# Orion-AI-Lab/KuroSiwo

Hardware: AMD Instinct MI355X
Metric: SAR tiles/sec (224x224, SNUNet-ECAM change-detection train step) (higher is better)
Workload: dtype bf16; 1 GPU; BASELINE.json configs[1]: SNUNet-ECAM CD, 2 dates x 2-ch GRD 224x224, per-GPU batch 32, ce+dice loss, Adam lr 1e-3, fwd+loss+bwd+optimizer; global_batch=32, base_channel=32, parallelism=dp1, hip_streams=3

## Files before the change

### include/ksmi.h

```cpp
#ifndef KSMI_H
#define KSMI_H
#include <stddef.h>
#include <stdint.h>

#ifdef __cplusplus
extern "C" {
#endif

#define KSMI_ABI_VERSION 7
#define KSMI_F32 0
#define KSMI_BF16 1
#define KSMI_E_ARG (-1)
#define KSMI_E_UNSUPPORTED (-2)
#define KSMI_MAX_SRC 6
#define KSMI_MAX_CHUNKS 72

int ksmi_abi_version(void);
const char* ksmi_last_error(void);
int ksmi_set_knob(const char* name, const char* value);
int ksmi_chunk_elems(int dtype);

#define KSMI_OP_CALL 0
#define KSMI_OP_ORDER 1
#define KSMI_OP_WAIT_SIDE 2
// ... 26 lines not shown
  int32_t n_begin;
  int32_t n_len;
  int32_t accumulate;
  int32_t pad_;
} ksmi_dst;

typedef struct ksmi_conv_desc {
  ksmi_src src[KSMI_MAX_SRC];
  ksmi_dst dst[KSMI_MAX_SRC];
  int32_t nsrc, ndst;
  const void* wpk;
  const float* bias;
  float* stats;
  const void* mask_src;
  const float* m_mean; const float* m_rstd; const float* m_scale; const float* m_shift;
  int32_t B, Hin, Win, Hout, Wout;
  int32_t KH, KW, stride, pad;
  int32_t TH, TW;
  int32_t N, Npad;
  int32_t nchunks;
  int32_t ps_cout;
  uint16_t chunk_c0[KSMI_MAX_CHUNKS];
  uint8_t chunk_src[KSMI_MAX_CHUNKS];
  int32_t pad_x;
  int32_t out_sy, out_sx, out_oy, out_ox, out_H, out_W;
  int32_t uniform_kc;
  int32_t in_sy, in_sx, in_oy, in_ox, in_H, in_W;
  float alpha;
  int32_t relu_out;
  int32_t residC;
  const void* resid;
  int32_t stats_rows;
  const void* gate_src; const void* xhat_src; const float* g_mean; const float* g_rstd;
  int32_t dir;
  int32_t pad2_;
} ksmi_conv_desc;


int ksmi_last_kernels(char* buf, int cap);
int ksmi_hbm_probe(int mode, const void* a, void* b, void* c, size_t nbytes, unsigned* sink, void* stream);
size_t ksmi_desc_size(int which);
int ksmi_conv_gate_supported(const ksmi_conv_desc* d, int dtype);
int ksmi_conv_grid_m(const ksmi_conv_desc* d);
int ksmi_conv_stats_rows(const ksmi_conv_desc* d, int dtype);
int ksmi_conv_forward(const ksmi_conv_desc* d, int dtype, void* stream);
int ksmi_conv_dispatch_info(const ksmi_conv_desc* d, int dtype, int32_t* info);

typedef struct ksmi_pack_desc {
  const float* w; void* out;
  int32_t nchunks, taps, N, Npad, n_mod;
  int64_t sK, sN, sD, sT;
  int32_t flip;
  int32_t k_off[KSMI_MAX_CHUNKS];
  int32_t k_len[KSMI_MAX_CHUNKS];
  int32_t use_tap_map;
  int32_t tap_map[16];
  int32_t uniform_kc, k_total;
} ksmi_pack_desc;
int ksmi_pack_weights(const ksmi_pack_desc* d, int dtype, void* stream);
int ksmi_pack_weights_batched(const ksmi_pack_desc* descs_device, int n, int dtype, void* stream);

typedef struct ksmi_wgrad_desc {
  ksmi_src src[KSMI_MAX_SRC];
  int32_t nsrc;
  const void* dy; int32_t dyC; int32_t dy_c_off;
  int32_t B, Hin, Win, Hout, Wout;
  int32_t KH, KW, stride, pad;
  int32_t TH, TW;
  int32_t N;
  int32_t nchunks;
  int32_t nsplit;
  float* partial;
  float* grad; int64_t gK, gN, gT; int32_t accumulate;
  int32_t k_off[KSMI_MAX_CHUNKS];
  int32_t k_len[KSMI_MAX_CHUNKS];
  uint16_t chunk_c0[KSMI_MAX_CHUNKS];
  uint8_t chunk_src[KSMI_MAX_CHUNKS];
  int32_t uniform_kc, k_total;
  int32_t in_sy, in_sx, in_oy, in_ox, in_H, in_W;
  int32_t pad_x_set, pad_x;
  int32_t use_tap_off;
  int32_t tap_off[16];
  float* bias_grad; int32_t bias_accumulate;
} ksmi_wgrad_desc;
size_t ksmi_conv_wgrad_workspace(const ksmi_wgrad_desc* d, int dtype);
int ksmi_conv_wgrad(const ksmi_wgrad_desc* d, int dtype, void* stream);
int ksmi_conv_wgrad_fuses_bias(const ksmi_wgrad_desc* d, int dtype);

int ksmi_conv_first_forward(const float* x_nchw, const float* w, const float* bias, void* out, float* stats,
                            int B, int Cin, int H, int W, int Cout, int dtype, void* stream);
int ksmi_conv_first_forward_raw(const float* x_nchw, const float* x_tail, int c_head, const float* w, const float* bias,
                                void* out, float* stats, int B, int Cin, int H, int W, int Cout, const float* mean,
                                const float* stdv, const float* clamp, int dtype, void* stream);
int ksmi_conv_first_stats_rows(int B, int H, int W);
int ksmi_im2col3x3(const float* x_nchw, void* out, int B, int Cin, int H, int W, int Kpad, int dtype, void* stream);
int ksmi_im2col3x3_raw(const float* x_nchw, const float* x_tail, int c_head, void* out, int B, int Cin, int H, int W,
                       int Kpad, const float* mean, const float* stdv, const float* clamp, int dtype, void* stream);
int ksmi_conv_first_wgrad(const float* x_nchw, const void* dy, float* dw, float* workspace, size_t ws_bytes,
                          int B, int Cin, int H, int W, int Cout, int accumulate, int dtype, void* stream);
size_t ksmi_conv_first_wgrad_workspace(int B, int Cin, int H, int W, int Cout);

int ksmi_bn_finalize(const float* partial, int rows, int Cpad, int C, double count,
                     const float* gamma, const float* beta, float* running_mean, float* running_var,
                     int64_t* num_batches_tracked, float momentum, float eps, int training,
                     float* mean, float* rstd, float* scale, float* shift, void* stream);
int ksmi_bn_add_relu(const void* z, const void* identity, const float* scale, const float* shift, void* out,
                     int64_t npix, int C, int dtype, void* stream);
int ksmi_bnrelu_bwd_reduce(const void* dout, const void* out, const void* z, const float* mean, const float* rstd,
                           float* partial, int rows, int64_t npix, int C, int dtype, void* stream);
int ksmi_reduce_rows(const float* partial, int rows, int K, int Cstride, int C, float* sums,
                     float* dgamma, float* dbeta, int accumulate, void* stream);
typedef struct ksmi_rowsum_desc {
  const float* partial;
  float* dst;
  int32_t rows, K, k, Cstride, C, accumulate;
  int32_t head, next;
} ksmi_rowsum_desc;
int ksmi_reduce_rows_batched(const ksmi_rowsum_desc* descs_device, int n, void* stream);
int ksmi_reduce_rows_batched_wide(const ksmi_rowsum_desc* descs_device, int n, int max_c, void* stream);
int ksmi_bnrelu_bwd_apply(void* dout_g, const void* out, const void* z, const float* mean, const float* rstd,
                          const float* gamma, const float* sums, void* dz, double count,
                          int64_t npix, int C, int dtype, void* stream);
int ksmi_bn_bwd_apply_gated(const void* g, const void* z, const float* mean, const float* rstd, const float* gamma, const float* sums,
                            void* dz, double count, int64_t npix, int C, int dtype, void* stream);
int ksmi_bn_bwd_apply_add(void* r_di, const void* g, const void* i, const float* mean, const float* rstd,
                          const float* gamma, const float* sums, float* partial, int rows, double count,
                          int64_t npix, int C, int dtype, void* stream);
int ksmi_bn_fused_supported(int C, int Cstride, int dtype);
int ksmi_bn_fused_max_rows(void);
int ksmi_bn_fin_add_relu(float* partial, int rows, int Cpad, int C, double count, const float* gamma, const float* beta,
                         float* running_mean, float* running_var, int64_t* num_batches_tracked, float momentum, float eps,
                         float* mean, float* rstd, float* scale, float* shift, const void* z, const void* identity, void* out,
                         void* pooled, int B, int H, int W, int dtype, void* stream);
int ksmi_bn_bwd_fin_apply_gated(float* partial, int rows, int Cstride, float* sums, float* dgamma, float* dbeta, int accumulate,
                                const void* g, const void* z, const float* mean, const float* rstd, const float* gamma, void* dz,
                                double count, int64_t npix, int C, int dtype, void* stream);
int ksmi_bnrelu_bwd_fin_apply(float* partial, int rows, int Cstride, float* sums, float* dgamma, float* dbeta, int accumulate,
                              void* dout_g, const void* out, const void* z, const float* mean, const float* rstd, const float* gamma,
                              void* dz, double count, int64_t npix, int C, int dtype, void* stream);
int ksmi_bn_bwd_fin_apply_add(float* partial, int rows, int Cstride, float* sums, float* dgamma, float* dbeta, int accumulate,
                              void* r_di, const void* g, const void* i, const float* mean, const float* rstd, const float* gamma,
                              float* bias_partial, int bias_rows, double count, int64_t npix, int C, int dtype, void* stream);
int ksmi_channel_sum(const void* x, float* partial, int rows, int64_t npix, int C, int dtype, void* stream);
int ksmi_colsum(const void* x, int64_t rows, int C, float* out, int accumulate, int dtype, void* stream);

int ksmi_maxpool2x2_forward(const void* x, void* y, int B, int H, int W, int C, int dtype, void* stream);
int ksmi_maxpool2x2_backward(const void* x, const void* dy, void* dx, int accumulate,
                             int B, int H, int W, int C, int dtype, void* stream);

int ksmi_ecam_pool(const void* const x[4], float* avg, float* mx, int32_t* argmax,
                   float* workspace, int B, int HW, int C, int dtype, void* stream);
size_t ksmi_ecam_pool_workspace(int B, int HW, int C);
int ksmi_ecam_mlp(const float* avg, const float* mx, const float* ca_fc1, const float* ca_fc2,
                  const float* ca1_fc1, const float* ca1_fc2, float* ca, float* ca1,
                  float* hidden , int B, int C, void* stream);
int ksmi_ecam_final_forward(const void* const x[4], const float* ca, const float* ca1, const float* wf,
                            const float* bias, float* logits, int B, int HW, int C, int ncls, int dtype, void* stream);
int ksmi_ecam_final_backward_reduce(const void* const x[4], const float* dlogits, const float* ca, const float* ca1,
                                    const float* wf, float* dca, float* dca1, float* dwf, float* dbias,
                                    float* workspace, int B, int HW, int C, int ncls, int dtype, void* stream);
size_t ksmi_ecam_bwd_workspace(int B, int HW, int C, int ncls);
int ksmi_ecam_mlp_backward(const float* avg, const float* mx, const float* hidden, const float* ca, const float* ca1,
                           const float* dca, const float* dca1, const float* ca_fc1, const float* ca_fc2,
                           const float* ca1_fc1, const float* ca1_fc2, float* davg, float* dmax,
                           float* g_ca_fc1, float* g_ca_fc2, float* g_ca1_fc1, float* g_ca1_fc2,
                           float* workspace, int B, int C, void* stream);
size_t ksmi_ecam_mlp_bwd_workspace(int B, int C);
int ksmi_ecam_final_backward_dx(void* const dx[4], const float* dlogits, const float* ca, const float* wf,
                                const float* davg, const float* dmax, const int32_t* argmax,
                                int B, int HW, int C, int ncls, int dtype, void* stream);

size_t ksmi_loss_workspace(int B, int HW);
int ksmi_ce_dice_forward(const float* logits, const int64_t* labels, const float* class_w, int with_dice,
                         float* out3, float* workspace, int B, int HW, int ignore_index, void* stream);
int ksmi_ce_dice_backward(const float* logits, const int64_t* labels, const float* class_w, int with_dice,
                          const float* workspace, const float* grad_scale ,
                          float* dlogits, int B, int HW, int ignore_index, void* stream);

#define KSMI_LOSS_DICE 1
#define KSMI_LOSS_LOVASZ 2
// ... 181 lines not shown
```

### kurosiwo_amd/_lib.py

```python
import ctypes as C
import os

_HERE = os.path.dirname(os.path.abspath(__file__))
LIB_PATH = os.path.join(_HERE, "libksmi.so")

KSMI_F32, KSMI_BF16 = 0, 1
LOSS_DICE, LOSS_LOVASZ, LOSS_FOCAL = 1, 2, 3
MAX_SRC, MAX_CHUNKS = 6, 72
ABI_VERSION = 7


class KsmiError(RuntimeError):
    pass


class Src(C.Structure):
    _fields_ = [("ptr", C.c_void_p), ("scale", C.c_void_p), ("shift", C.c_void_p),
                ("C", C.c_int32), ("c_off", C.c_int32), ("c_len", C.c_int32), ("relu", C.c_int32)]


class Dst(C.Structure):
    _fields_ = [("ptr", C.c_void_p), ("C", C.c_int32), ("c_off", C.c_int32), ("n_begin", C.c_int32),
                ("n_len", C.c_int32), ("accumulate", C.c_int32), ("pad_", C.c_int32)]


class ConvDesc(C.Structure):
    _fields_ = [("src", Src * MAX_SRC), ("dst", Dst * MAX_SRC), ("nsrc", C.c_int32), ("ndst", C.c_int32),
                ("wpk", C.c_void_p), ("bias", C.c_void_p), ("stats", C.c_void_p),
                ("mask_src", C.c_void_p), ("m_mean", C.c_void_p), ("m_rstd", C.c_void_p),
                ("m_scale", C.c_void_p), ("m_shift", C.c_void_p),
                ("B", C.c_int32), ("Hin", C.c_int32), ("Win", C.c_int32), ("Hout", C.c_int32), ("Wout", C.c_int32),
                ("KH", C.c_int32), ("KW", C.c_int32), ("stride", C.c_int32), ("pad", C.c_int32),
                ("TH", C.c_int32), ("TW", C.c_int32), ("N", C.c_int32), ("Npad", C.c_int32),
                ("nchunks", C.c_int32), ("ps_cout", C.c_int32),
                ("chunk_c0", C.c_uint16 * MAX_CHUNKS), ("chunk_src", C.c_uint8 * MAX_CHUNKS),
                ("pad_x", C.c_int32), ("out_sy", C.c_int32), ("out_sx", C.c_int32), ("out_oy", C.c_int32),
                ("out_ox", C.c_int32), ("out_H", C.c_int32), ("out_W", C.c_int32),
                ("uniform_kc", C.c_int32), ("in_sy", C.c_int32), ("in_sx", C.c_int32), ("in_oy", C.c_int32), ("in_ox", C.c_int32),
                ("in_H", C.c_int32), ("in_W", C.c_int32), ("alpha", C.c_float), ("relu_out", C.c_int32), ("residC", C.c_int32),
                ("resid", C.c_void_p), ("stats_rows", C.c_int32),
                ("gate_src", C.c_void_p), ("xhat_src", C.c_void_p), ("g_mean", C.c_void_p), ("g_rstd", C.c_void_p),
                ("dir", C.c_int32), ("pad2_", C.c_int32)]


class PackDesc(C.Structure):
    _fields_ = [("w", C.c_void_p), ("out", C.c_void_p),
                ("nchunks", C.c_int32), ("taps", C.c_int32), ("N", C.c_int32), ("Npad", C.c_int32), ("n_mod", C.c_int32),
                ("sK", C.c_int64), ("sN", C.c_int64), ("sD", C.c_int64), ("sT", C.c_int64),
                ("flip", C.c_int32),
                ("k_off", C.c_int32 * MAX_CHUNKS), ("k_len", C.c_int32 * MAX_CHUNKS),
                ("use_tap_map", C.c_int32), ("tap_map", C.c_int32 * 16), ("uniform_kc", C.c_int32), ("k_total", C.c_int32)]


class TiffInfo(C.Structure):
    _fields_ = [(k, C.c_int32) for k in ("width", "height", "bands", "bits", "sample_format", "compression", "predictor", "tiled",
                                         "big_endian", "bigtiff", "has_geo", "has_nodata")] + [
        ("pixel_scale", C.c_double * 2), ("origin", C.c_double * 2), ("tie_pixel", C.c_double * 2), ("nodata", C.c_double)]


class RowsumDesc(C.Structure):
    _fields_ = [("partial", C.c_void_p), ("dst", C.c_void_p), ("rows", C.c_int32), ("K", C.c_int32), ("k", C.c_int32),
                ("Cstride", C.c_int32), ("C", C.c_int32), ("accumulate", C.c_int32), ("head", C.c_int32), ("next", C.c_int32)]


class WgradDesc(C.Structure):
    _fields_ = [("src", Src * MAX_SRC), ("nsrc", C.c_int32),
                ("dy", C.c_void_p), ("dyC", C.c_int32), ("dy_c_off", C.c_int32),
                ("B", C.c_int32), ("Hin", C.c_int32), ("Win", C.c_int32), ("Hout", C.c_int32), ("Wout", C.c_int32),
                ("KH", C.c_int32), ("KW", C.c_int32), ("stride", C.c_int32), ("pad", C.c_int32),
                ("TH", C.c_int32), ("TW", C.c_int32), ("N", C.c_int32), ("nchunks", C.c_int32), ("nsplit", C.c_int32),
                ("partial", C.c_void_p), ("grad", C.c_void_p),
                ("gK", C.c_int64), ("gN", C.c_int64), ("gT", C.c_int64), ("accumulate", C.c_int32),
                ("k_off", C.c_int32 * MAX_CHUNKS), ("k_len", C.c_int32 * MAX_CHUNKS),
                ("chunk_c0", C.c_uint16 * MAX_CHUNKS), ("chunk_src", C.c_uint8 * MAX_CHUNKS),
                ("uniform_kc", C.c_int32), ("k_total", C.c_int32),
                ("in_sy", C.c_int32), ("in_sx", C.c_int32), ("in_oy", C.c_int32), ("in_ox", C.c_int32), ("in_H", C.c_int32), ("in_W", C.c_int32),
                ("pad_x_set", C.c_int32), ("pad_x", C.c_int32), ("use_tap_off", C.c_int32), ("tap_off", C.c_int32 * 16),
                ("bias_grad", C.c_void_p), ("bias_accumulate", C.c_int32)]


class Op(C.Structure):
    _fields_ = [(k, C.c_int32) for k in ("kind", "sig", "lane", "side", "tag", "a", "b", "nargs")] + [("fn", C.c_void_p), ("args", C.c_void_p)]


OP_CALL, OP_ORDER, OP_WAIT_SIDE = 0, 1, 2

_vp, _i, _i64, _f, _d, _sz = C.c_void_p, C.c_int, C.c_int64, C.c_float, C.c_double, C.c_size_t
_P4 = C.c_void_p * 4

SIGNATURES = {
    "ksmi_abi_version": (_i, []),
    "ksmi_last_kernels": (_i, [C.c_char_p, _i]),
    "ksmi_hbm_probe": (_i, [_i, _vp, _vp, _vp, C.c_size_t, _vp, _vp]),
    "ksmi_last_error": (C.c_char_p, []),
    "ksmi_set_knob": (_i, [C.c_char_p, C.c_char_p]),
    "ksmi_thunk_id": (_i, [C.c_char_p]),
    "ksmi_runner_create": (_vp, []),
    "ksmi_runner_destroy": (_i, [_vp]),
    "ksmi_runner_set_streams": (_i, [_vp, _vp, _vp, _vp, _vp]),
    "ksmi_run_list": (_i, [_vp, _vp, _i, _i, _vp, C.POINTER(C.c_int32)]),
    "ksmi_runner_join": (_i, [_vp]),
    "ksmi_conv_dispatch_info": (_i, [C.POINTER(ConvDesc), _i, C.POINTER(C.c_int32)]),
    "ksmi_chunk_elems": (_i, [_i]),
    "ksmi_conv_grid_m": (_i, [C.POINTER(ConvDesc)]),
    "ksmi_conv_forward": (_i, [C.POINTER(ConvDesc), _i, _vp]),
    "ksmi_pack_weights": (_i, [C.POINTER(PackDesc), _i, _vp]),
    "ksmi_pack_weights_batched": (_i, [_vp, _i, _i, _vp]),
    "ksmi_conv_wgrad_workspace": (_sz, [C.POINTER(WgradDesc), _i]),
    "ksmi_conv_wgrad": (_i, [C.POINTER(WgradDesc), _i, _vp]),
    "ksmi_conv_wgrad_fuses_bias": (_i, [C.POINTER(WgradDesc), _i]),
    "ksmi_conv_stats_rows": (_i, [C.POINTER(ConvDesc), _i]),
    "ksmi_conv_gate_supported": (_i, [C.POINTER(ConvDesc), _i]),
    "ksmi_desc_size": (C.c_size_t, [_i]),
    "ksmi_conv_first_forward": (_i, [_vp, _vp, _vp, _vp, _vp, _i, _i, _i, _i, _i, _i, _vp]),
    "ksmi_conv_first_forward_raw": (_i, [_vp, _vp, _i, _vp, _vp, _vp, _vp, _i, _i, _i, _i, _i, _vp, _vp, _vp, _i, _vp]),
    "ksmi_conv_first_stats_rows": (_i, [_i, _i, _i]),
    "ksmi_im2col3x3": (_i, [_vp, _vp, _i, _i, _i, _i, _i, _i, _vp]),
    "ksmi_im2col3x3_raw": (_i, [_vp, _vp, _i, _vp, _i, _i, _i, _i, _i, _vp, _vp, _vp, _i, _vp]),
    "ksmi_conv_first_wgrad": (_i, [_vp, _vp, _vp, _vp, _sz, _i, _i, _i, _i, _i, _i, _i, _vp]),
    "ksmi_conv_first_wgrad_workspace": (_sz, [_i, _i, _i, _i, _i]),
    "ksmi_bn_finalize": (_i, [_vp, _i, _i, _i, _d, _vp, _vp, _vp, _vp, _vp, _f, _f, _i, _vp, _vp, _vp, _vp, _vp]),
    "ksmi_bn_add_relu": (_i, [_vp, _vp, _vp, _vp, _vp, _i64, _i, _i, _vp]),
    "ksmi_bn_fused_supported": (_i, [_i, _i, _i]),
    "ksmi_bn_fused_max_rows": (_i, []),
    "ksmi_bn_fin_add_relu": (_i, [_vp, _i, _i, _i, _d, _vp, _vp, _vp, _vp, _vp, _f, _f, _vp, _vp, _vp, _vp, _vp, _vp, _vp, _vp, _i, _i, _i, _i, _vp]),
    "ksmi_bn_bwd_fin_apply_gated": (_i, [_vp, _i, _i, _vp, _vp, _vp, _i, _vp, _vp, _vp, _vp, _vp, _vp, _d, _i64, _i, _i, _vp]),
    "ksmi_bnrelu_bwd_fin_apply": (_i, [_vp, _i, _i, _vp, _vp, _vp, _i, _vp, _vp, _vp, _vp, _vp, _vp, _vp, _d, _i64, _i, _i, _vp]),
    "ksmi_bn_bwd_fin_apply_add": (_i, [_vp, _i, _i, _vp, _vp, _vp, _i, _vp, _vp, _vp, _vp, _vp, _vp, _vp, _i, _d, _i64, _i, _i, _vp]),
    "ksmi_bnrelu_bwd_reduce": (_i, [_vp, _vp, _vp, _vp, _vp, _vp, _i, _i64, _i, _i, _vp]),
    "ksmi_reduce_rows": (_i, [_vp, _i, _i, _i, _i, _vp, _vp, _vp, _i, _vp]),
    "ksmi_reduce_rows_batched": (_i, [_vp, _i, _vp]),
    "ksmi_reduce_rows_batched_wide": (_i, [_vp, _i, _i, _vp]),
    "ksmi_bnrelu_bwd_apply": (_i, [_vp, _vp, _vp, _vp, _vp, _vp, _vp, _vp, _d, _i64, _i, _i, _vp]),
    "ksmi_bn_bwd_apply_gated": (_i, [_vp, _vp, _vp, _vp, _vp, _vp, _vp, _d, _i64, _i, _i, _vp]),
    "ksmi_bn_bwd_apply_add": (_i, [_vp, _vp, _vp, _vp, _vp, _vp, _vp, _vp, _i, _d, _i64, _i, _i, _vp]),
    "ksmi_channel_sum": (_i, [_vp, _vp, _i, _i64, _i, _i, _vp]),
    "ksmi_colsum": (_i, [_vp, _i64, _i, _vp, _i, _i, _vp]),
    "ksmi_gather_rows": (_i, [_vp, _vp, _i, _vp, _vp, _i, _i, _i, _i, _i, _i, _vp]),
    "ksmi_scatter_rows": (_i, [_vp, _vp, _vp, _i, _vp, _vp, _i, _i, _i, _i, _i, _vp]),
    "ksmi_batch_sum": (_i, [_vp, _vp, _i, _i64, _i, _i, _vp]),
    "ksmi_mse_workspace": (C.c_size_t, []),
    "ksmi_mse_loss": (_i, [_vp, _vp, _vp, _f, _vp, _vp, _vp, _i64, _i, _vp]),
    "ksmi_maxpool2x2_forward": (_i, [_vp, _vp, _i, _i, _i, _i, _i, _vp]),
    "ksmi_maxpool2x2_backward": (_i, [_vp, _vp, _vp, _i, _i, _i, _i, _i, _i, _vp]),
    "ksmi_ecam_pool": (_i, [_P4, _vp, _vp, _vp, _vp, _i, _i, _i, _i, _vp]),
    "ksmi_ecam_pool_workspace": (_sz, [_i, _i, _i]),
    "ksmi_ecam_mlp": (_i, [_vp, _vp, _vp, _vp, _vp, _vp, _vp, _vp, _vp, _i, _i, _vp]),
    "ksmi_ecam_final_forward": (_i, [_P4, _vp, _vp, _vp, _vp, _vp, _i, _i, _i, _i, _i, _vp]),
    "ksmi_ecam_final_backward_reduce": (_i, [_P4, _vp, _vp, _vp, _vp, _vp, _vp, _vp, _vp, _vp, _i, _i, _i, _i, _i, _vp]),
    "ksmi_ecam_bwd_workspace": (_sz, [_i, _i, _i, _i]),
    "ksmi_ecam_mlp_backward": (_i, [_vp] * 18 + [_i, _i, _vp]),
    "ksmi_ecam_mlp_bwd_workspace": (_sz, [_i, _i]),
    "ksmi_ecam_final_backward_dx": (_i, [_P4, _vp, _vp, _vp, _vp, _vp, _vp, _i, _i, _i, _i, _i, _vp]),
    "ksmi_loss_workspace": (_sz, [_i, _i]),
    "ksmi_ce_dice_forward": (_i, [_vp, _vp, _vp, _i, _vp, _vp, _i, _i, _i, _vp]),
    "ksmi_ce_dice_backward": (_i, [_vp, _vp, _vp, _i, _vp, _vp, _vp, _i, _i, _i, _vp]),
    "ksmi_seg_loss_workspace": (_sz, [_i, _i, _i]),
    "ksmi_seg_loss_forward": (_i, [_i, _vp, _vp, _vp, _f, _vp, _vp, _i, _i, _i, _vp]),
    "ksmi_seg_loss_backward": (_i, [_i, _vp, _vp, _vp, _f, _vp, _vp, _vp, _i, _i, _i, _vp]),
    "ksmi_argmax_confusion": (_i, [_vp, _vp, _vp, _vp, _i, _i, _i, _i, _vp]),
    "ksmi_argmax_confusion_grouped": (_i, [_vp, _vp, _vp, _vp, _vp, _vp, _vp, _vp, _i, _i, _i, _i, _vp]),
    "ksmi_adam_step": (_i, [_vp, _vp, _vp, _vp, _i64, _vp, _f, _f, _f, _f, _f, _f, _vp]),
    "ksmi_adamw_step": (_i, [_vp, _vp, _vp, _vp, _i64, _vp, _f, _f, _f, _f, _f, _f, _vp]),
    "ksmi_adam_step_mirror": (_i, [_vp, _vp, _vp, _vp, _i64, _vp, _f, _f, _f, _f, _f, _f, _i, _vp, _vp]),
    "ksmi_sgd_step": (_i, [_vp, _vp, _vp, _i64, _vp, _f, _f, _f, _f, _vp]),
    "ksmi_layernorm_forward": (_i, [_vp, _vp, _vp, _vp, _vp, _vp, _i, _i, _f, _i, _vp]),
    "ksmi_layernorm_bwd_blocks": (_i, [_i]),
    "ksmi_layernorm_backward": (_i, [_vp, _vp, _vp, _vp, _vp, _vp, _i, _vp, _i, _i, _i, _vp]),
    "ksmi_gelu_forward": (_i, [_vp, _vp, _i64, _i, _vp]),
    "ksmi_gelu_backward": (_i, [_vp, _vp, _vp, _i64, _i, _vp]),
    "ksmi_add": (_i, [_vp, _vp, _vp, _i64, _i, _vp]),
    "ksmi_relu_backward": (_i, [_vp, _vp, _vp, _i64, _i, _vp]),
    "ksmi_relu_forward": (_i, [_vp, _vp, _i64, _i, _vp]),
    "ksmi_sar_preprocess": (_i, [_vp, _vp, _vp, _vp, _i, _i, _i64, C.c_float, _vp]),
    "ksmi_augment_views": (_i, [_vp, _vp, _vp, _vp, _vp, _vp, _i, _i, _i, _i, _f, C.c_uint32, _f, _f, C.c_uint32, _f, _f, C.c_uint32, _i, _i, _i, _i, _vp, _vp]),
    "ksmi_augment_masks": (_i, [_vp, _vp, _vp, _vp, _vp, _i, _i, _i, _i, _vp]),
    "ksmi_bmm_f32": (_i, [_vp, _vp, _vp, _vp, _i, _i, _i, _i, _i, C.POINTER(C.c_int64), C.POINTER(C.c_int64), C.POINTER(C.c_int64), C.c_float, _i, _vp]),
    "ksmi_softmax_rows_f32": (_i, [_vp, _vp, _i64, _i, C.c_float, _vp]),
    "ksmi_softmax_rows_backward_f32": (_i, [_vp, _vp, _vp, _i64, _i, C.c_float, _vp]),
    "ksmi_semantic_tokens_forward": (_i, [_vp, _vp, _vp, _vp, _vp, _i, _i, _i, _i, _i, _i, _vp]),
    "ksmi_semantic_tokens_backward": (_i, [_vp, _vp, _vp, _vp, _vp, _vp, _i, _i, _i, _i, _i, _i, _i, _vp]),
    "ksmi_token_cross_forward": (_i, [_vp, _vp, _vp, _vp, _vp, _vp, _vp, _i, _i, _i, _i, _i, _i, C.c_float, _i, _vp]),
    "ksmi_token_cross_bwd_workspace": (_sz, [_i, _i, _i]),
    "ksmi_token_cross_backward": (_i, [_vp, _vp, _vp, _vp, _vp, _vp, _vp, _vp, _vp, _vp, _vp, _i, _i, _vp, _i, _i, _i, _i, _i, _i, C.c_float, _i, _vp]),
    "ksmi_tiff_info_read": (_i, [C.c_char_p, C.POINTER(TiffInfo)]),
    "ksmi_tiff_read_f32": (_i, [C.c_char_p, _vp, _i64, C.POINTER(TiffInfo)]),
    "ksmi_tiff_read_native": (_i, [C.c_char_p, _vp, _i64, C.POINTER(TiffInfo)]),
    "ksmi_tile_batch_read": (_i, [C.POINTER(C.c_char_p), _i, _vp, _i, _i, _i]),
    "ksmi_tile_batch_read_bands": (_i, [C.POINTER(C.c_char_p), _i, _vp, _i, _i, _i, _i]),
    "ksmi_tiles_fill_nodata": (_i, [_vp, _i, _i, _i, _i]),
    "ksmi_cast_bf16": (_i, [_vp, _vp, _i64, _vp]),
    "ksmi_up_gemm_supported": (_i, [_i, _i, _i, _i, _i]),
    "ksmi_up_wgrad_supported": (_i, [_i, _i, _i, _i, _i]),
    "ksmi_up_pack_weight": (_i, [_vp, _vp, _i, _vp]),
    "ksmi_up_pack_weights_batched": (_i, [_vp, _vp, _vp, _i, _vp]),
    "ksmi_up_forward": (_i, [_vp, _vp, _vp, _vp, _i, _i, _i, _i, _vp]),
    "ksmi_up_dgrad": (_i, [_vp, _vp, _vp, _i, _i, _i, _i, _i, _vp]),
    "ksmi_up_wgrad_workspace": (C.c_size_t, [_i, _i, _i, _i]),
    "ksmi_up_wgrad": (_i, [_vp, _vp, _vp, _vp, _i, _i, _i, _i, _i, _vp]),
    "ksmi_gemm_nt": (_i, [_vp, _i, _vp, _i, _vp, _vp, _i, _vp, _i, _i, _i, _i, _vp]),
    "ksmi_gemm_nn": (_i, [_vp, _i, _vp, _i, _vp, _i, _i, _i, _i, _i, _vp]),
# ... 114 lines not shown
```

### kurosiwo_amd/csrc/elementwise.hip

```cpp
#include <stdlib.h>
#include "common.h"
#include "../../include/ksmi.h"
#include "errors.h"

namespace {

constexpr int kThreads = 256;

struct ChanWalk {
  int cv, pl, npl, active;
  __device__ ChanWalk(int CV) {
    npl = kThreads / CV; if (npl < 1) npl = 1;
    active = (int)threadIdx.x < npl * CV && CV <= kThreads;
    cv = threadIdx.x % CV; pl = threadIdx.x / CV;
  }
};

template <int K, int VEC>
__device__ __forceinline__ void block_channel_reduce(const float* val, const ChanWalk& w, int CV, int C, float* partial, int row) {
  __shared__ float red[kThreads * 2];
#pragma unroll
  for (int k = 0; k < K; ++k) {
#pragma unroll
    for (int j0 = 0; j0 < VEC; j0 += 2) {
// ... 450 lines not shown
  for (int c = 0; c < CIN; ++c)
#pragma unroll
    for (int t = 0; t < 9; ++t) xin[c * 9 + t] = xs[c * 324 + (ly + t / 3) * 18 + lx + t % 3];
  for (int n0 = 0; n0 < Cout; n0 += NC) {
    const int nc = min(NC, Cout - n0);
    for (int i = tid; i < nc * KTP; i += 256) { const int j = i / KTP, k = i - j * KTP; wl[i] = k < KT ? w[(n0 + j) * KT + k] : 0.f; }
    if (tid < nc) wl[NC * KTP + tid] = bias ? bias[n0 + tid] : 0.f;
    __syncthreads();
#pragma unroll 4
    for (int j = 0; j < nc; ++j) {
      float a = wl[NC * KTP + j];
      float wr[KTP];
#pragma unroll
      for (int k = 0; k < KTP; k += 4) *(f32x4*)(wr + k) = *(const f32x4*)(wl + j * KTP + k);
#pragma unroll
      for (int k = 0; k < KT; ++k) a = fmaf(xin[k], wr[k], a);
      ot[tid * OP + j] = ok ? ElemTraits<T>::cvt(a) : 0.f;
    }
    __syncthreads();
    if (stats) {
      const int n = tid & (NC - 1), grp = tid / NC;
      if (n < nc) {
        float sm = 0.f, sq = 0.f;
#pragma unroll 8
        for (int i = 0; i < NC; ++i) { const float v = ot[(grp * NC + i) * OP + n]; sm += v; sq += v * v; }
        red[(grp * 2 + 0) * NC + n] = sm; red[(grp * 2 + 1) * NC + n] = sq;
      }
    }
    const int vpp = nc / VEC;
    for (int v = tid; v < 256 * vpp; v += 256) {
      const int p = v / vpp, q = v - p * vpp;
      const int py = ty * 16 + (p >> 4), px = tx * 16 + (p & 15);
      if (py >= H || px >= W) continue;
      float o[VEC];
#pragma unroll
      for (int j = 0; j < VEC; ++j) o[j] = ot[p * OP + q * VEC + j];
      *(u32x4*)(out + (((int64_t)b * H + py) * W + px) * Cout + n0 + q * VEC) = vec_pack<T>(o);
    }
    __syncthreads();
    if (stats && tid < 2 * nc) {
      const int which = tid / nc, n = tid - which * nc;
      float t = 0.f;
#pragma unroll
      for (int g = 0; g < G; ++g) t += red[(g * 2 + which) * NC + n];
      stats[((size_t)blockIdx.x * 2 + which) * Cout + n0 + n] = t;
    }
  }
}

template <typename T>
__global__ __launch_bounds__(256) void im2col3x3_kernel(const float* __restrict__ x, T* out, int B, int Cin, int H, int W, int Kpad,
                                                        const float* __restrict__ nmean, const float* __restrict__ nstd,
                                                        const float* __restrict__ nclamp, const float* __restrict__ xtail, int chead) {
  constexpr int VEC = ElemTraits<T>::kVec;
  extern __shared__ __attribute__((aligned(16))) unsigned char smem[];
  float* xs = (float*)smem;
  const int tilesX = (W + 15) / 16, tilesY = (H + 15) / 16;
  int bm = blockIdx.x;
  const int tx = bm % tilesX; bm /= tilesX;
  const int ty = bm % tilesY; const int b = bm / tilesY;
  const int tid = threadIdx.x;
  for (int i = tid; i < Cin * 324; i += 256) {
    const int c = i / 324, r = i - c * 324, hy = r / 18, hx = r - hy * 18;
    const int iy = ty * 16 - 1 + hy, ix = tx * 16 - 1 + hx;
    float v = 0.f;
    if (iy >= 0 && iy < H && ix >= 0 && ix < W) v = raw_tile_value(image_value(x, xtail, chead, Cin, b, c, H, W, iy, ix), c, nmean, nstd, nclamp);
    xs[i] = v;
  }
  __syncthreads();
  const int KV = Kpad / VEC;
  for (int v = tid; v < 256 * KV; v += 256) {
    const int p = v / KV, q = v - p * KV;
    const int ly = p >> 4, lx = p & 15;
    const int oy = ty * 16 + ly, ox = tx * 16 + lx;
    if (oy >= H || ox >= W) continue;
    float f[VEC];
#pragma unroll
    for (int j = 0; j < VEC; ++j) {
      const int k = q * VEC + j;
      const int c = k / 9, t = k - c * 9;
      f[j] = c < Cin ? xs[c * 324 + (ly + t / 3) * 18 + lx + t % 3] : 0.f;
    }
    *(u32x4*)(out + (((int64_t)b * H + oy) * W + ox) * Kpad + q * VEC) = vec_pack<T>(f);
  }
}

template <typename T>
__global__ __launch_bounds__(256) void conv_first_wgrad_kernel(const float* x, const T* dy, float* partial,
                                                               int B, int Cin, int H, int W, int Cout) {
  extern __shared__ __attribute__((aligned(16))) unsigned char smem[];
  float* xs = (float*)smem;
  float* dys = xs + Cin * 324;
  const int tilesX = (W + 15) / 16, tilesY = (H + 15) / 16;
  const int patches = B * tilesX * tilesY;
  const int tid = threadIdx.x;
  const int KT = Cin * 9;
  const int n = tid % Cout, grp = tid / Cout, ngrp = 256 / Cout;
  constexpr int MAXK = 12;
  float acc[MAXK];
#pragma unroll
  for (int j = 0; j < MAXK; ++j) acc[j] = 0.f;
  const int ldy = Cout + 1;
  for (int patch = blockIdx.x; patch < patches; patch += gridDim.x) {
    int bm = patch;
    const int tx = bm % tilesX; bm /= tilesX;
    const int ty = bm % tilesY; const int b = bm / tilesY;
    __syncthreads();
    for (int i = tid; i < Cin * 324; i += 256) {
      const int c = i / 324, r = i - c * 324, hy = r / 18, hx = r - hy * 18;
      const int iy = ty * 16 - 1 + hy, ix = tx * 16 - 1 + hx;
      xs[i] = (iy >= 0 && iy < H && ix >= 0 && ix < W) ? x[(((int64_t)b * Cin + c) * H + iy) * W + ix] : 0.f;
    }
    for (int i = tid; i < 256 * Cout; i += 256) {
      const int p = i / Cout, nn = i - p * Cout;
      const int oy = ty * 16 + (p >> 4), ox = tx * 16 + (p & 15);
      dys[p * ldy + nn] = (oy < H && ox < W) ? ElemTraits<T>::ld(dy + (((int64_t)b * H + oy) * W + ox) * Cout + nn) : 0.f;
    }
    __syncthreads();
    for (int p = 0; p < 256; ++p) {
      const float g = dys[p * ldy + n];
      const int ly = p >> 4, lx = p & 15;
#pragma unroll
      for (int j = 0; j < MAXK; ++j) {
        const int k = grp + j * ngrp;
        if (k < KT) {
          const int c = k / 9, t = k - c * 9;
          acc[j] += g * xs[c * 324 + (ly + t / 3) * 18 + lx + t % 3];
        }
      }
    }
  }
#pragma unroll
  for (int j = 0; j < MAXK; ++j) {
    const int k = grp + j * ngrp;
    if (k < KT) partial[((size_t)blockIdx.x * Cout + n) * KT + k] = acc[j];
  }
}

__global__ void sum_rows_flat_kernel(const float* partial, int rows, int64_t n, float* out, int accumulate) {
  for (int64_t i = (int64_t)blockIdx.x * blockDim.x + threadIdx.x; i < n; i += (int64_t)gridDim.x * blockDim.x) {
    double s = 0.0;
    for (int r = 0; r < rows; ++r) s += (double)partial[(size_t)r * n + i];
    out[i] = accumulate ? out[i] + (float)s : (float)s;
  }
}

__global__ void step_increment_kernel(int64_t* step) { if (threadIdx.x == 0 && blockIdx.x == 0) *step += 1; }

template <bool DECOUPLED, bool MIRROR = false>
__global__ void adam_kernel(float* p, const float* g, float* m, float* v, int64_t n, const int64_t* step,
                            float lr, float b1, float b2, float eps, float wd, float gscale, bf16_t* mirror = nullptr) {
  const double t = (double)*step;
  const float bc1 = (float)(1.0 - pow((double)b1, t));
  const float bc2s = (float)sqrt(1.0 - pow((double)b2, t));
  const float step_size = lr / bc1;
  auto upd = [&](float gi, float& pi, float& mi, float& vi) {
    gi *= gscale;
    if (DECOUPLED) pi = pi * (1.f - lr * wd);
    else if (wd != 0.f) gi += wd * pi;
    mi = mi + (gi - mi) * (1.f - b1);
    vi = vi * b2 + gi * gi * (1.f - b2);
    const float denom = sqrtf(vi) / bc2s + eps;
    pi = pi - step_size * (mi / denom);
  };
  const bool vec = ((((uintptr_t)p | (uintptr_t)g | (uintptr_t)m | (uintptr_t)v) & 15) == 0);
  const int64_t nv = vec ? n / 4 : 0;
// ... 318 lines not shown

int ksmi_conv_first_stats_rows(int B, int H, int W) { return B * ((H + 15) / 16) * ((W + 15) / 16); }

static int first_conv_sources(const float* xtail, int* chead, int Cin, const float* nmean, const float* nstd, const float* nclamp) {
  if ((nmean != nullptr) != (nstd != nullptr) || (nmean != nullptr) != (nclamp != nullptr))
    return ksmi_fail(KSMI_E_ARG, "conv_first: mean, std and clamp come together");
  if (xtail == nullptr) *chead = Cin;
  else if (*chead < 1 || *chead >= Cin) return ksmi_fail(KSMI_E_ARG, "conv_first: a tail image needs 1 <= c_head < Cin");
  return 0;
}

int ksmi_conv_first_forward_raw(const float* x, const float* xtail, int chead, const float* w, const float* bias, void* out, float* stats,
                                int B, int Cin, int H, int W, int Cout, const float* nmean, const float* nstd, const float* nclamp,
                                int dtype, void* stream) {
  if (int rc = first_conv_sources(xtail, &chead, Cin, nmean, nstd, nclamp)) return rc;
  const int vec = dtype == KSMI_BF16 ? 8 : 4;
  if (Cin < 1 || Cin > 8 || Cout % vec || Cout > 256) return ksmi_fail(KSMI_E_ARG, "conv_first: Cin<=8, Cout multiple of vector, <=256");
  const int grid = ksmi_conv_first_stats_rows(B, H, W);
  const size_t lds = (size_t)(Cin * 324 + 256 * 17 + 512 + 16 * ((Cin * 9 + 3) / 4 * 4) + 16) * sizeof(float);
  hipStream_t st = (hipStream_t)stream;
#define KSMI_CF(CIN_)                                                                                                     \
  case CIN_:                                                                                                              \
    if (dtype == KSMI_BF16) hipLaunchKernelGGL((conv_first_fwd_kernel<bf16_t, CIN_>), dim3(grid), dim3(256), lds, st, x, w, bias, (bf16_t*)out, stats, B, H, W, Cout, nmean, nstd, nclamp, xtail, chead); \
    else hipLaunchKernelGGL((conv_first_fwd_kernel<float, CIN_>), dim3(grid), dim3(256), lds, st, x, w, bias, (float*)out, stats, B, H, W, Cout, nmean, nstd, nclamp, xtail, chead);                    \
    break;
  if (dtype != KSMI_BF16 && dtype != KSMI_F32) return ksmi_fail(KSMI_E_ARG, "bad dtype");
  switch (Cin) { KSMI_CF(1) KSMI_CF(2) KSMI_CF(3) KSMI_CF(4) KSMI_CF(5) KSMI_CF(6) KSMI_CF(7) KSMI_CF(8) }
#undef KSMI_CF
  return ksmi_check_launch("conv_first_fwd");
}

int ksmi_conv_first_forward(const float* x, const float* w, const float* bias, void* out, float* stats, int B, int Cin, int H,
                            int W, int Cout, int dtype, void* stream) {
  return ksmi_conv_first_forward_raw(x, nullptr, Cin, w, bias, out, stats, B, Cin, H, W, Cout, nullptr, nullptr, nullptr, dtype, stream);
}

static int conv_first_wgrad_blocks(int B, int H, int W) {
  const int patches = B * ((H + 15) / 16) * ((W + 15) / 16);
  return patches < 512 ? patches : 512;
}

size_t ksmi_conv_first_wgrad_workspace(int B, int Cin, int H, int W, int Cout) {
  return (size_t)conv_first_wgrad_blocks(B, H, W) * Cout * Cin * 9 * sizeof(float);
}

int ksmi_conv_first_wgrad(const float* x, const void* dy, float* dw, float* workspace, size_t ws_bytes, int B, int Cin, int H,
                          int W, int Cout, int accumulate, int dtype, void* stream) {
  if (Cin < 1 || Cin > 8 || 256 % Cout || (Cin * 9 + 256 / Cout - 1) / (256 / Cout) > 12)
    return ksmi_fail(KSMI_E_ARG, "conv_first_wgrad: unsupported Cin/Cout");
  if (ws_bytes < ksmi_conv_first_wgrad_workspace(B, Cin, H, W, Cout)) return ksmi_fail(KSMI_E_ARG, "conv_first_wgrad: workspace too small");
  const int blocks = conv_first_wgrad_blocks(B, H, W);
  const size_t lds = (size_t)(Cin * 324 + 256 * (Cout + 1)) * sizeof(float);
  KSMI_DT(dtype,
          {
            auto k = conv_first_wgrad_kernel<bf16_t>;
            if (lds > 65536) (void)hipFuncSetAttribute((const void*)k, hipFuncAttributeMaxDynamicSharedMemorySize, (int)lds);
            hipLaunchKernelGGL(k, dim3(blocks), dim3(256), lds, (hipStream_t)stream, x, (const bf16_t*)dy, workspace, B, Cin, H, W, Cout);
          },
          {
            auto k = conv_first_wgrad_kernel<float>;
            if (lds > 65536) (void)hipFuncSetAttribute((const void*)k, hipFuncAttributeMaxDynamicSharedMemorySize, (int)lds);
            hipLaunchKernelGGL(k, dim3(blocks), dim3(256), lds, (hipStream_t)stream, x, (const float*)dy, workspace, B, Cin, H, W, Cout);
          });
  int rc = ksmi_check_launch("conv_first_wgrad");
  if (rc) return rc;
  const int64_t n = (int64_t)Cout * Cin * 9;
  hipLaunchKernelGGL(sum_rows_flat_kernel, dim3(grid_for(n)), dim3(256), 0, (hipStream_t)stream, workspace, blocks, n, dw, accumulate);
  return ksmi_check_launch("conv_first_wgrad_reduce");
}

int ksmi_im2col3x3_raw(const float* x_nchw, const float* xtail, int chead, void* out, int B, int Cin, int H, int W, int Kpad,
                       const float* nmean, const float* nstd, const float* nclamp, int dtype, void* stream) {
  if (int rc = first_conv_sources(xtail, &chead, Cin, nmean, nstd, nclamp)) return rc;
  const int vec = dtype == KSMI_BF16 ? 8 : 4;
  if (Cin < 1 || Cin * 9 > Kpad || Kpad % vec || Cin > 32) return ksmi_fail(KSMI_E_ARG, "im2col3x3: need Cin*9 <= Kpad, Kpad multiple of the vector");
  const int grid = B * ((H + 15) / 16) * ((W + 15) / 16);
  const size_t lds = (size_t)Cin * 324 * sizeof(float);
  KSMI_DT(dtype,
          hipLaunchKernelGGL(im2col3x3_kernel<bf16_t>, dim3(grid), dim3(256), lds, (hipStream_t)stream, x_nchw, (bf16_t*)out, B, Cin, H, W, Kpad, nmean, nstd, nclamp, xtail, chead),
          hipLaunchKernelGGL(im2col3x3_kernel<float>, dim3(grid), dim3(256), lds, (hipStream_t)stream, x_nchw, (float*)out, B, Cin, H, W, Kpad, nmean, nstd, nclamp, xtail, chead));
  return ksmi_check_launch("im2col3x3");
}

int ksmi_im2col3x3(const float* x_nchw, void* out, int B, int Cin, int H, int W, int Kpad, int dtype, void* stream) {
  return ksmi_im2col3x3_raw(x_nchw, nullptr, Cin, out, B, Cin, H, W, Kpad, nullptr, nullptr, nullptr, dtype, stream);
}

int ksmi_adam_step(float* p, const float* g, float* m, float* v, int64_t n, int64_t* step_count, float lr, float beta1,
                   float beta2, float eps, float weight_decay, float grad_scale, void* stream) {
  if (!p || !g || !m || !v || !step_count || n < 0) return ksmi_fail(KSMI_E_ARG, "adam: bad args");
  hipLaunchKernelGGL(step_increment_kernel, dim3(1), dim3(64), 0, (hipStream_t)stream, step_count);
  hipLaunchKernelGGL((adam_kernel<false, false>), dim3(grid_for((n + 3) / 4, 8192)), dim3(256), 0, (hipStream_t)stream, p, g, m, v, n, step_count, lr, beta1,
                     beta2, eps, weight_decay, grad_scale, (bf16_t*)nullptr);
  return ksmi_check_launch("adam");
}

int ksmi_adam_step_mirror(float* p, const float* g, float* m, float* v, int64_t n, int64_t* step_count, float lr, float beta1,
                          float beta2, float eps, float weight_decay, float grad_scale, int decoupled, void* mirror_bf16, void* stream) {
  if (!p || !g || !m || !v || !step_count || !mirror_bf16 || n < 0 || ((uintptr_t)mirror_bf16 & 7)) return ksmi_fail(KSMI_E_ARG, "adam_mirror: bad args");
  hipLaunchKernelGGL(step_increment_kernel, dim3(1), dim3(64), 0, (hipStream_t)stream, step_count);
  if (decoupled)
    hipLaunchKernelGGL((adam_kernel<true, true>), dim3(grid_for((n + 3) / 4, 8192)), dim3(256), 0, (hipStream_t)stream, p, g, m, v, n, step_count, lr, beta1,
                       beta2, eps, weight_decay, grad_scale, (bf16_t*)mirror_bf16);
  else
    hipLaunchKernelGGL((adam_kernel<false, true>), dim3(grid_for((n + 3) / 4, 8192)), dim3(256), 0, (hipStream_t)stream, p, g, m, v, n, step_count, lr, beta1,
                       beta2, eps, weight_decay, grad_scale, (bf16_t*)mirror_bf16);
  return ksmi_check_launch("adam_mirror");
}

int ksmi_adamw_step(float* p, const float* g, float* m, float* v, int64_t n, int64_t* step_count, float lr, float beta1,
                    float beta2, float eps, float weight_decay, float grad_scale, void* stream) {
  if (!p || !g || !m || !v || !step_count || n < 0) return ksmi_fail(KSMI_E_ARG, "adamw: bad args");
  hipLaunchKernelGGL(step_increment_kernel, dim3(1), dim3(64), 0, (hipStream_t)stream, step_count);
  hipLaunchKernelGGL((adam_kernel<true, false>), dim3(grid_for((n + 3) / 4, 8192)), dim3(256), 0, (hipStream_t)stream, p, g, m, v, n, step_count, lr, beta1,
                     beta2, eps, weight_decay, grad_scale, (bf16_t*)nullptr);
  return ksmi_check_launch("adamw");
}

int ksmi_sgd_step(float* p, const float* g, float* mom, int64_t n, int64_t* step_count, float lr, float momentum,
                  float weight_decay, float grad_scale, void* stream) {
  if (!p || !g || !step_count || (momentum != 0.f && !mom)) return ksmi_fail(KSMI_E_ARG, "sgd: bad args");
  hipLaunchKernelGGL(step_increment_kernel, dim3(1), dim3(64), 0, (hipStream_t)stream, step_count);
  hipLaunchKernelGGL(sgd_kernel, dim3(grid_for(n, 4096)), dim3(256), 0, (hipStream_t)stream, p, g, mom, n, step_count, lr, momentum,
                     weight_decay, grad_scale);
  return ksmi_check_launch("sgd");
}

int ksmi_fill_zero(void* p, size_t bytes, void* stream) {
  hipError_t e = hipMemsetAsync(p, 0, bytes, (hipStream_t)stream);
  if (e != hipSuccess) return ksmi_fail((int)e, hipGetErrorString(e));
  return 0;
}

int ksmi_nchw_to_nhwc(const float* x, void* y, int B, int C, int HW, int dtype, void* stream) {
  const int64_t n = (int64_t)B * C * HW;
  KSMI_DT(dtype,
          hipLaunchKernelGGL(nchw_to_nhwc_kernel<bf16_t>, dim3(grid_for(n, 8192)), dim3(256), 0, (hipStream_t)stream, x, (bf16_t*)y, B, C, HW),
          hipLaunchKernelGGL(nchw_to_nhwc_kernel<float>, dim3(grid_for(n, 8192)), dim3(256), 0, (hipStream_t)stream, x, (float*)y, B, C, HW));
  return ksmi_check_launch("nchw_to_nhwc");
}

int ksmi_nhwc_to_nchw(const void* x, float* y, int B, int C, int HW, int dtype, void* stream) {
  const int64_t n = (int64_t)B * C * HW;
  KSMI_DT(dtype,
          hipLaunchKernelGGL(nhwc_to_nchw_kernel<bf16_t>, dim3(grid_for(n, 8192)), dim3(256), 0, (hipStream_t)stream, (const bf16_t*)x, y, B, C, HW),
          hipLaunchKernelGGL(nhwc_to_nchw_kernel<float>, dim3(grid_for(n, 8192)), dim3(256), 0, (hipStream_t)stream, (const float*)x, y, B, C, HW));
  return ksmi_check_launch("nhwc_to_nchw");
}

int ksmi_selftest_mma(const void* a, const void* b, float* c, int dtype, void* stream) {
  KSMI_DT(dtype,
          hipLaunchKernelGGL(selftest_mma_kernel<bf16_t>, dim3(1), dim3(64), 0, (hipStream_t)stream, (const bf16_t*)a, (const bf16_t*)b, c),
          hipLaunchKernelGGL(selftest_mma_kernel<float>, dim3(1), dim3(64), 0, (hipStream_t)stream, (const float*)a, (const float*)b, c));
  return ksmi_check_launch("selftest_mma");
}

int ksmi_selftest_tr16(const uint16_t* in256, uint16_t* out256, void* stream) {
  hipLaunchKernelGGL(selftest_tr16_kernel, dim3(1), dim3(64), 0, (hipStream_t)stream, in256, out256);
  return ksmi_check_launch("selftest_tr16");
}

}
```

### kurosiwo_amd/csrc/igemm.hip

```cpp
#include <stdio.h>
#include <stdlib.h>
#include "common.h"
#include "../../include/ksmi.h"
#include "errors.h"
#include "igemm_epilogue.h"
#include "wgrad3.h"
#include "igemm3.h"
#include "igemm4.h"

namespace {


template <typename T, int NT, int KH, int KW>
__global__ __launch_bounds__(256) void igemm_fwd_kernel(const ksmi_conv_desc d) {
  constexpr int TAPS = KH * KW;
  constexpr int BN = NT * 16;
  constexpr int VEC = ElemTraits<T>::kVec;
  constexpr int KC = VEC * 4;
  extern __shared__ __attribute__((aligned(16))) unsigned char smem[];

  const int tid = threadIdx.x, lane = tid & 63, wave = tid >> 6;
  const int g = lane >> 4, l15 = lane & 15;

  const int tilesX = (d.Wout + d.TW - 1) / d.TW, tilesY = (d.Hout + d.TH - 1) / d.TH;
// ... 690 lines not shown
static bool wgrad_generic_forced() { static const bool on = ksmi_knob_is_set("KSMI_WGRAD_GENERIC"); return on; }
static bool gemm_tn_eligible(const ksmi_wgrad_desc* d, int es) {
  return es == 2 && d->KH == 1 && d->KW == 1 && d->stride == 1 && d->pad == 0 && d->nsrc == 1 && d->src[0].scale == nullptr &&
         d->Hin == d->Hout && d->Win == d->Wout && (d->src[0].c_len % 8) == 0 && (d->N % 8) == 0 && d->N >= 64 && d->src[0].c_len >= 64 &&
         !wgrad_generic_forced();
}
static void gemm_tn_geom(const ksmi_wgrad_desc* d, int kc, int& nsplit, int& rps, int& tk, int& tn, int& bt) {
  const int rows = d->B * d->Hout * d->Wout;
  const int K = d->nchunks * kc;
  const int npad = (d->N + 15) & ~15;
  tk = (K + 127) / 128; tn = (npad + 127) / 128;
  bool plain = d->gK == 1 && (!d->use_tap_off || d->tap_off[0] == 0) && d->gN >= d->src[0].c_len && d->gN < ((int64_t)1 << 31);
  if (plain && !d->uniform_kc)
    for (int i = 0; i < d->nchunks; ++i) plain = plain && d->k_off[i] == i * kc;
  const int steps_all = (rows + 63) / 64;
  double best = 1e30; int bs = 1; bt = 128;
  static const int f_bt = ksmi_knob_int("KSMI_TN_BT", 0), f_s = ksmi_knob_int("KSMI_TN_SPLIT", 0);
  for (int b = 128; b >= 64; b -= 32) {
    if (f_bt && b != f_bt) continue;
    const double step_us = b == 128 ? 0.95 : b == 96 ? 0.78 : 0.6;
    for (int s = 1; s <= 256 && s <= steps_all; s = s < 8 ? s + 1 : s * 2) {
      if (s == 1 && !plain) continue;
      if (f_s && s != f_s) continue;
      const int acols = s == 1 ? K : npad, bcols = s == 1 ? npad : K;
      const int tiles = ((acols + 127) / 128) * ((bcols + b - 1) / b);
      const int steps = (steps_all + s - 1) / s;
      const int rounds = (tiles * s + 255) / 256;
      const bool spl = ksmi_gemm2_tn_spl(tiles * s, steps);
      double t = rounds * ((spl ? 0.73 : 1.0) * steps * step_us + (spl ? 4.0 : 3.0));
      if (s > 1) t += 2.0 * s * (double)K * npad * 4.0 / 4.0e6 + 3.0 + 0.08 * (s > 16 ? 16 + (s - 16) / 8 : s);
      if (t < best) { best = t; bs = s; bt = b; }
    }
  }
  rps = ((steps_all + bs - 1) / bs) * 64;
  nsplit = (rows + rps - 1) / rps;
}

struct WgradGeom { int taps, kc, nt, bn, patches, pps, nsplit, ntiles, npad; size_t lds; bool tn; int rps, tk, tnn, tbt; bool v3; ksmi_wgrad3_geom_t g3; };

template <typename T>
WgradGeom wgrad_geom(const ksmi_wgrad_desc* d) {
  WgradGeom g;
  g.taps = d->KH * d->KW;
  g.kc = ElemTraits<T>::kVec * 4;
  g.npad = (d->N + 15) & ~15;
  g.nt = g.npad >= 64 ? 4 : (g.npad >= 32 ? 2 : 1);
  static const int wnt_cap = ksmi_knob_int("KSMI_WGRAD_NT", 4);
  if (g.nt > wnt_cap) g.nt = wnt_cap;
  static const bool wnt4 = ksmi_knob_is_set("KSMI_WGRAD_NT4");
  if (g.taps >= 9 && g.nt > 2 && !wnt4) g.nt = 2;
  g.bn = g.nt * 16;
  g.ntiles = (g.npad + g.bn - 1) / g.bn;
  const int tilesX = (d->Wout + d->TW - 1) / d->TW, tilesY = (d->Hout + d->TH - 1) / d->TH;
  g.patches = d->B * tilesX * tilesY;
  static const int wg_target = ksmi_knob_int("KSMI_WGRAD_WGS", 1024);
  static const int split_cap = ksmi_knob_int("KSMI_WGRAD_SPLITS", 512);
  int want = wg_target / (d->nchunks * g.ntiles);
  if (want < 1) want = 1;
  if (want > split_cap) want = split_cap;
  if (want > g.patches) want = g.patches;
  g.pps = (g.patches + want - 1) / want;
  g.nsplit = (g.patches + g.pps - 1) / g.pps;
  const int HH = (d->TH - 1) * d->stride + d->KH, HW = (d->TW - 1) * d->stride + d->KW;
  const int P = d->TH * d->TW, Ppad = (P + g.kc - 1) / g.kc * g.kc;
  g.lds = ((HH * HW * 64 + 255) & ~255) + (size_t)Ppad * g.bn * sizeof(T);
  if (g.taps == 1 && g.lds < (size_t)(g.kc / 16) * g.nt * 4096) g.lds = (size_t)(g.kc / 16) * g.nt * 4096;
  g.tn = gemm_tn_eligible(d, (int)sizeof(T));
  if (g.tn) gemm_tn_geom(d, g.kc, g.nsplit, g.rps, g.tk, g.tnn, g.tbt);
  g.v3 = !g.tn && ksmi_wgrad3_geom(d, sizeof(T) == 2 ? KSMI_BF16 : KSMI_F32, &g.g3);
  if (g.v3) g.nsplit = g.g3.nsplit;
  return g;
}

static bool wgrad_slab_bias_on() {
  static const bool on = (ksmi_knob_int("KSMI_SLAB_BIAS", 1) != 0);
  return on;
}

template <typename T>
int launch_wgrad(const ksmi_wgrad_desc* d, hipStream_t st) {
  WgradGeom g = wgrad_geom<T>(d);
  if (d->TH * d->TW > 256) return ksmi_fail(KSMI_E_ARG, "wgrad: patch too large");
  if (d->nsplit != g.nsplit) return ksmi_fail(KSMI_E_ARG, "wgrad: nsplit does not match ksmi_conv_wgrad_workspace geometry");
  if (g.v3) {
    int rc3 = ksmi_wgrad3_launch(d, &g.g3, st);
    if (rc3) return rc3;
    return ksmi_wgrad3_reduce(d, &g.g3, st);
  }
  if (g.tn) {
    bool plain = d->gK == 1 && (!d->use_tap_off || d->tap_off[0] == 0) && d->gN >= d->src[0].c_len && d->gN < ((int64_t)1 << 31);
    if (plain && !d->uniform_kc)
      for (int i = 0; i < d->nchunks; ++i) plain = plain && d->k_off[i] == i * g.kc;
    {
      const int rows = d->B * d->Hout * d->Wout;
      const bool direct = plain && g.nsplit == 1;
      const int r2 = ksmi_gemm2_tn((const bf16_t*)d->src[0].ptr + d->src[0].c_off, d->src[0].C, (const bf16_t*)d->dy + d->dy_c_off, d->dyC, d->partial,
                                   g.npad, direct ? d->grad : nullptr, d->gN, rows, d->src[0].c_len, d->N, d->nchunks * g.kc, g.nsplit, g.rps,
                                   g.tbt, d->accumulate, (direct || (plain && wgrad_slab_bias_on())) ? d->bias_grad : nullptr, d->bias_accumulate, st);
      if (r2 < 0) return r2;
      if (r2 == 0) {
        if (direct) return 0;
        if (g.nsplit > 16) {
          const size_t totalr = (size_t)d->nchunks * g.kc * g.npad;
          int blocksr = (int)((totalr * 8 + 255) / 256); if (blocksr > 4096) blocksr = 4096;
          hipLaunchKernelGGL(wgrad_reduce_kernel, dim3(blocksr), dim3(256), 0, st, *d, 1, g.kc);
          return ksmi_check_launch("wgrad_reduce");
        }
        static const int tr_on = ksmi_knob_int("KSMI_TN_REDUCE_TR", 1);
        if (tr_on && plain) {
          const int Kreal = d->uniform_kc ? d->k_total : d->k_off[d->nchunks - 1] + d->k_len[d->nchunks - 1];
          const dim3 gridr((g.npad + 31) / 32, (Kreal + 31) / 32);
          hipLaunchKernelGGL(tn_reduce_tr_kernel, gridr, dim3(256), 0, st, d->partial, g.nsplit, (size_t)d->nchunks * g.kc * g.npad, g.npad, d->N, Kreal,
                             d->grad, d->gN, d->accumulate);
          return ksmi_check_launch("tn_reduce_tr");
        }
        const size_t total0 = (size_t)d->nchunks * g.kc * g.npad / 4;
        int blocks0 = (int)((total0 + 255) / 256); if (blocks0 > 8192) blocks0 = 8192;
        hipLaunchKernelGGL(tn_reduce_kernel, dim3(blocks0), dim3(256), 0, st, *d, g.kc, d->nchunks * g.kc);
        return ksmi_check_launch("tn_reduce");
      }
    }
    hipLaunchKernelGGL(gemm_tn_wgrad_kernel, dim3(g.tk, g.tnn, g.nsplit), dim3(256), 0, st, *d, d->B * d->Hout * d->Wout, g.rps, d->nchunks * g.kc);
    int rc0 = ksmi_check_launch("gemm_tn_wgrad");
    if (rc0) return rc0;
    if (g.nsplit > 16) {
      const size_t totalr = (size_t)d->nchunks * g.kc * g.npad;
      int blocksr = (int)((totalr * 8 + 255) / 256); if (blocksr > 4096) blocksr = 4096;
      hipLaunchKernelGGL(wgrad_reduce_kernel, dim3(blocksr), dim3(256), 0, st, *d, 1, g.kc);
      return ksmi_check_launch("wgrad_reduce");
    }
    const size_t total0 = (size_t)d->nchunks * g.kc * g.npad / 4;
    int blocks0 = (int)((total0 + 255) / 256); if (blocks0 > 8192) blocks0 = 8192;
    hipLaunchKernelGGL(tn_reduce_kernel, dim3(blocks0), dim3(256), 0, st, *d, g.kc, d->nchunks * g.kc);
    return ksmi_check_launch("tn_reduce");
  }
  {
    const size_t pin = d->in_sy ? (size_t)d->B * d->in_H * d->in_W : (size_t)d->B * d->Hin * d->Win;
    size_t cmax = d->dyC;
    for (int i = 0; i < d->nsrc; ++i) if ((size_t)d->src[i].C > cmax) cmax = d->src[i].C;
    const size_t pmax = pin > (size_t)d->B * d->Hout * d->Wout ? pin : (size_t)d->B * d->Hout * d->Wout;
    if (pmax * cmax * sizeof(T) >= ((size_t)1 << 32)) return ksmi_fail(KSMI_E_UNSUPPORTED, "wgrad: a tensor of 4 GiB or more is not supported");
  }
  static const int wdbg = ksmi_knob_int("KSMI_WDBG", 0);
  const dim3 grid(g.nsplit, d->nchunks, g.ntiles);
  static const bool lin_off = ksmi_knob_is_set("KSMI_WGRAD_NOLIN");
  const bool lin = !lin_off && sizeof(T) == 2 && (16 % d->TW) == 0 && ((d->TH * d->TW) % 32) == 0;
#define KSMI_LAUNCH_WG(NT_, KH_, KW_)                                                               \
  do {                                                                                              \
    if (lin) {                                                                                      \
      auto kfn = igemm_wgrad_kernel<T, NT_, KH_, KW_, true>; KSMI_NOTE(kfn);                                        \
      if (g.lds > 65536) (void)hipFuncSetAttribute((const void*)kfn, hipFuncAttributeMaxDynamicSharedMemorySize, (int)g.lds); \
      hipLaunchKernelGGL(kfn, grid, dim3(256), g.lds, st, *d, g.patches, g.pps, wdbg);              \
    } else {                                                                                        \
      auto kfn = igemm_wgrad_kernel<T, NT_, KH_, KW_, false>; KSMI_NOTE(kfn);                                       \
      if (g.lds > 65536) (void)hipFuncSetAttribute((const void*)kfn, hipFuncAttributeMaxDynamicSharedMemorySize, (int)g.lds); \
      hipLaunchKernelGGL(kfn, grid, dim3(256), g.lds, st, *d, g.patches, g.pps, wdbg);              \
    }                                                                                               \
  } while (0)
#define KSMI_DISPATCH_WNT(KH_, KW_)                                                                 \
  switch (g.nt) {                                                                                   \
    case 1: KSMI_LAUNCH_WG(1, KH_, KW_); break;                                                     \
    case 2: KSMI_LAUNCH_WG(2, KH_, KW_); break;                                                     \
    default: KSMI_LAUNCH_WG(4, KH_, KW_); break;                                                    \
  }
  if (d->KH == 3 && d->KW == 3) { KSMI_DISPATCH_WNT(3, 3) }
  else if (d->KH == 1 && d->KW == 1) { KSMI_DISPATCH_WNT(1, 1) }
// ... 55 lines not shown
int ksmi_conv_dispatch_info(const ksmi_conv_desc* d, int dtype, int32_t* info) {
  if (!d || !info) return ksmi_fail(KSMI_E_ARG, "conv_dispatch_info: null argument");
  for (int i = 0; i < 8; ++i) info[i] = 0;
  static const bool force_v1 = ksmi_knob_is_set("KSMI_IGEMM_V1");
  ksmi_igemm3_geom_t g3;
  if (!force_v1 && !d->gate_src && ksmi_igemm3_geom(d, dtype, &g3) && (d->stats == nullptr || d->stats_rows == g3.gx)) {
    info[0] = 3; info[1] = 1; info[6] = g3.gx; info[7] = g3.gy;
    return 0;
  }
  ksmi_igemm4_geom_t g4;
  if (!force_v1 && ksmi_igemm4_geom(d, dtype, &g4) && (d->stats == nullptr || d->stats_rows == g4.gx)) {
    info[0] = 4; info[1] = ksmi_igemm4_launchable(d, &g4) ? 1 : 0;
    info[2] = g4.WM; info[3] = g4.NF; info[4] = g4.nwv; info[5] = g4.deep; info[6] = g4.gx; info[7] = g4.gy;
    return 0;
  }
  info[0] = (!force_v1 && ksmi_igemm2_eligible(d, dtype)) ? 2 : 1;
  info[1] = 1;
  return 0;
}

int ksmi_conv_forward(const ksmi_conv_desc* d, int dtype, void* stream) {
  if (!d || d->nsrc < 1 || d->nsrc > KSMI_MAX_SRC || d->ndst < 1 || d->ndst > KSMI_MAX_SRC || d->nchunks < 1 ||
      (d->nchunks > KSMI_MAX_CHUNKS && !(d->uniform_kc && d->nsrc == 1)))
    return ksmi_fail(KSMI_E_ARG, "conv: bad descriptor");
  if (dtype != KSMI_BF16 && dtype != KSMI_F32) return ksmi_fail(KSMI_E_ARG, "conv: bad dtype");
  static const bool force_v1 = ksmi_knob_is_set("KSMI_IGEMM_V1");
  {
    ksmi_igemm3_geom_t g3;
    if (!force_v1 && !d->gate_src && ksmi_igemm3_geom(d, dtype, &g3) && (d->stats == nullptr || d->stats_rows == g3.gx))
      return ksmi_igemm3_launch(d, &g3, (hipStream_t)stream);
    ksmi_igemm4_geom_t g4;
    if (!force_v1 && ksmi_igemm4_geom(d, dtype, &g4) && (d->stats == nullptr || d->stats_rows == g4.gx))
      return ksmi_igemm4_launch(d, &g4, (hipStream_t)stream);
    if (d->gate_src) return ksmi_fail(KSMI_E_UNSUPPORTED, "conv: the gate epilogue needs the persistent long-K kernel (ksmi_conv_gate_supported)");
  }
  if (d->stats && d->stats_rows != 0 && d->stats_rows != ksmi_conv_grid_m(d))
    return ksmi_fail(KSMI_E_ARG, "conv: stats_rows does not match the kernel this descriptor runs on (set it from ksmi_conv_stats_rows)");
  if (!force_v1 && ksmi_igemm2_eligible(d, dtype)) return ksmi_igemm2_launch(d, dtype, (hipStream_t)stream);
  if (d->alpha != 0.f || d->resid || d->relu_out || d->uniform_kc)
    return ksmi_fail(KSMI_E_UNSUPPORTED, "conv: alpha/resid/relu_out/uniform chunks need whole-chunk sources (igemm2 path)");
  if (dtype == KSMI_BF16) return launch_fwd<bf16_t>(d, (hipStream_t)stream);
  return launch_fwd<float>(d, (hipStream_t)stream);
}

int ksmi_pack_weights(const ksmi_pack_desc* d, int dtype, void* stream) {
  if (!d || d->nchunks < 1 || (d->nchunks > KSMI_MAX_CHUNKS && !d->uniform_kc)) return ksmi_fail(KSMI_E_ARG, "pack: bad descriptor");
  const int kc = ksmi_chunk_elems(dtype);
  const size_t total = (size_t)d->nchunks * d->taps * d->Npad * kc;
  int blocks = (int)((total + 255) / 256); if (blocks > 4096) blocks = 4096;
  if (dtype == KSMI_BF16) hipLaunchKernelGGL(pack_weights_kernel<bf16_t>, dim3(blocks), dim3(256), 0, (hipStream_t)stream, *d);
  else hipLaunchKernelGGL(pack_weights_kernel<float>, dim3(blocks), dim3(256), 0, (hipStream_t)stream, *d);
  return ksmi_check_launch("pack_weights");
}

int ksmi_pack_weights_batched(const ksmi_pack_desc* descs_device, int n, int dtype, void* stream) {
  if (!descs_device || n < 1) return ksmi_fail(KSMI_E_ARG, "pack_batched: bad args");
  static const int gx = ksmi_knob_int("KSMI_PACK_GRID", 512);
  const dim3 grid(gx < 1 ? 1 : gx, n);
  if (dtype == KSMI_BF16) hipLaunchKernelGGL(pack_weights_batched_kernel<bf16_t>, grid, dim3(256), 0, (hipStream_t)stream, descs_device);
  else if (dtype == KSMI_F32) hipLaunchKernelGGL(pack_weights_batched_kernel<float>, grid, dim3(256), 0, (hipStream_t)stream, descs_device);
  else return ksmi_fail(KSMI_E_ARG, "pack_batched: bad dtype");
  return ksmi_check_launch("pack_weights_batched");
}

size_t ksmi_conv_wgrad_workspace(const ksmi_wgrad_desc* d, int dtype) {
  WgradGeom g = dtype == KSMI_BF16 ? wgrad_geom<bf16_t>(d) : wgrad_geom<float>(d);
  return (size_t)g.nsplit * g.taps * d->nchunks * g.kc * g.npad * sizeof(float);
}

int ksmi_conv_wgrad_fuses_bias(const ksmi_wgrad_desc* d, int dtype) {
  if (!d || dtype != KSMI_BF16 || d->nsrc != 1) return 0;
  static const bool off = ksmi_knob_is_set("KSMI_NO_FUSED_BIAS_GRAD");
  if (off) return 0;
  WgradGeom g = wgrad_geom<bf16_t>(d);
  if (!g.tn || g.v3) return 0;
  bool plain = d->gK == 1 && (!d->use_tap_off || d->tap_off[0] == 0) && d->gN >= d->src[0].c_len && d->gN < ((int64_t)1 << 31);
  if (plain && !d->uniform_kc)
    for (int i = 0; i < d->nchunks; ++i) plain = plain && d->k_off[i] == i * g.kc;
  if (!(plain && ksmi_gemm2_tn_enabled(d->src[0].c_len, d->N, g.rps))) return 0;
  if (g.nsplit == 1) return 1;
  return wgrad_slab_bias_on() && (g.tbt == 64 || g.tbt == 96 || g.tbt == 128) ? 2 : 0;
}

int ksmi_conv_wgrad(const ksmi_wgrad_desc* d, int dtype, void* stream) {
  if (!d || d->nsrc < 1 || d->nsrc > KSMI_MAX_SRC || d->nchunks < 1 || (d->nchunks > KSMI_MAX_CHUNKS && !(d->uniform_kc && d->nsrc == 1)))
    return ksmi_fail(KSMI_E_ARG, "wgrad: bad descriptor");
  if (dtype == KSMI_BF16) return launch_wgrad<bf16_t>(d, (hipStream_t)stream);
  if (dtype == KSMI_F32) return launch_wgrad<float>(d, (hipStream_t)stream);
  return ksmi_fail(KSMI_E_ARG, "wgrad: bad dtype");
}

}
```

### kurosiwo_amd/csrc/wgrad3.h

```cpp
#pragma once
#include <hip/hip_runtime.h>
#include "../../include/ksmi.h"

struct ksmi_wgrad3_geom_t {
  int TH, TW, HWc, tilesX, tilesY;
  int WC, NTL;
  int KT, NTt;
  int patches, pps, nsplit;
  int xpl, stage;
  int nst;
  int r0, c0;
  size_t lds;
};
bool ksmi_wgrad3_geom(const ksmi_wgrad_desc* d, int dtype, ksmi_wgrad3_geom_t* g);
int ksmi_wgrad3_launch(const ksmi_wgrad_desc* d, const ksmi_wgrad3_geom_t* g, hipStream_t st);
int ksmi_wgrad3_reduce(const ksmi_wgrad_desc* d, const ksmi_wgrad3_geom_t* g, hipStream_t st);
```

### kurosiwo_amd/csrc/wgrad3.hip

```cpp
#include <stdlib.h>
#include "common.h"
#include "../../include/ksmi.h"
#include "errors.h"
#include "igemm_epilogue.h"
#include "wgrad3.h"
#include "dma.h"

namespace {

struct Wg3Args {
  ksmi_wgrad_desc d;
  int TH, TW, HWc, HPv;
  int xpl, stage;
  int tilesX, tilesY, patches, pps;
  int KT, NTt;
  uint32_t m_hw, m_tw, m_tx, m_ty, m_tiles, m_ntt;
  int kstride;
  int hymask;
  int lds_bytes;
  int nst;
  const unsigned char* zero;
};

__device__ __attribute__((aligned(64))) unsigned char wg3_zero_page[64];
KSMI_DEVICE_SYMBOL_GETTER(wg3_zero, wg3_zero_page)

__device__ __forceinline__ u32x4 tr_frag(unsigned a0, unsigned a1) {
  const s16x4 lo = __builtin_amdgcn_ds_read_tr16_b64_v4i16((__attribute__((address_space(3))) s16x4*)(uintptr_t)a0);
  const s16x4 hi = __builtin_amdgcn_ds_read_tr16_b64_v4i16((__attribute__((address_space(3))) s16x4*)(uintptr_t)a1);
  return __builtin_bit_cast(u32x4, __builtin_shufflevector(lo, hi, 0, 1, 2, 3, 4, 5, 6, 7));
}

__device__ __forceinline__ int wg_chunk_c0(const ksmi_wgrad_desc& d, int ch) {
  if (d.uniform_kc) return ch * d.uniform_kc;
  const uint32_t w = ((const uint32_t*)d.chunk_c0)[ch >> 1];
  return (ch & 1) ? (int)(w >> 16) : (int)(w & 0xffffu);
}
__device__ __forceinline__ int wg_chunk_src(const ksmi_wgrad_desc& d, int ch) {
  if (d.uniform_kc) return 0;
  return (int)((((const uint32_t*)d.chunk_src)[ch >> 2] >> ((ch & 3) * 8)) & 0xffu);
}

template <int WC, int WN, int NF, bool AFF, bool DEEP, int R0 = -1, int C0 = -1, bool PART = false>
__global__ __launch_bounds__(256, 2) void wgrad3_kernel(const Wg3Args ka) {
  typedef bf16_t T;
  const ksmi_wgrad_desc& d = ka.d;
  constexpr bool SUB = R0 >= 0;
  constexpr int NTAP = SUB ? 4 : 9;
  static_assert(!SUB || (R0 <= 1 && C0 >= 0 && C0 <= 1), "2 x 2 window inside the 3 x 3 neighbourhood");
  constexpr int CPT = WC / 2;
  constexpr int NFT = WN * NF;
  constexpr int NPL = (NFT + 1) / 2;
  constexpr int NTL = NFT * 16;
  constexpr int XIT = 4;
  extern __shared__ __attribute__((aligned(16))) unsigned char smem[];

  const int tid = threadIdx.x, lane = tid & 63;
  const int wave = __builtin_amdgcn_readfirstlane(tid >> 6);
  const int cfi = wave % WC, wn = wave / WC;
  const int g = lane >> 4, l15 = lane & 15;

  const int L = (int)xcd_remap(blockIdx.x, gridDim.x);
  const FastDiv dTiles(ka.KT * ka.NTt, ka.m_tiles), dNTt(ka.NTt, ka.m_ntt);
  const int split = dTiles.div(L);
  const int rem = L - split * (ka.KT * ka.NTt);
  const int kt = dNTt.div(rem), nt = rem - kt * ka.NTt;
  const int n0 = nt * NTL;
  const int TW = ka.TW, TH = ka.TH, HWc = ka.HWc;
  const int P = TH * TW;
  const FastDiv dHW(HWc, ka.m_hw), dTW(TW, ka.m_tw), dTX(ka.tilesX, ka.m_tx), dTY(ka.tilesY, ka.m_ty);
  const int xpl = ka.xpl, stage = ka.stage;

  const unsigned char* sp[CPT];
  uint32_t cb[CPT];
  bool cvalid[CPT];
  int cc0[CPT], klen[CPT], krem[CPT];
#pragma unroll
  for (int c = 0; c < CPT; ++c) {
    const int ch = kt * CPT + c;
    cvalid[c] = ch < d.nchunks;
    const int chs = cvalid[c] ? ch : 0;
    const ksmi_src& sr = d.src[wg_chunk_src(d, chs)];
    cc0[c] = wg_chunk_c0(d, chs);
    sp[c] = (const unsigned char*)((const T*)sr.ptr + sr.c_off + cc0[c]);
    cb[c] = (uint32_t)sr.C * 2u;
    krem[c] = PART ? sr.c_len - cc0[c] : 32;
    klen[c] = krem[c] >= 32 ? 32 : ((krem[c] + 7) & ~7);
  }
  const unsigned char* const dyp = (const unsigned char*)((const T*)d.dy + d.dy_c_off);
  const uint32_t dycb = (uint32_t)d.dyC * 2u;

  for (int i = tid * 16; i < ka.lds_bytes; i += 256 * 16) *(u32x4*)(smem + i) = (u32x4){0u, 0u, 0u, 0u};
  float* aff_tab = (float*)(smem + ka.nst * stage);
  if constexpr (AFF) {
    __syncthreads();
    if (tid < CPT * 32) {
      const int c = tid >> 5, j = tid & 31;
      const ksmi_src& sr = d.src[0];
      const bool ok = cvalid[c] && (!PART || j < krem[c]);
      aff_tab[tid * 2 + 0] = ok ? sr.scale[cc0[c] + j] : 0.f;
      aff_tab[tid * 2 + 1] = ok ? sr.shift[cc0[c] + j] : 0.f;
    }
  }
  const bool aff_relu = AFF && d.src[0].relu != 0;

  const unsigned lds0 = (unsigned)(uintptr_t)smem;
  unsigned a_tab[2][3][2], b_tab[NF][2];
#pragma unroll
  for (int h = 0; h < 2; ++h) {
    const int p0 = g * 8 + h * 4 + (l15 >> 2);
    const int ly = dTW.div(p0), lx = p0 - ly * TW;
#pragma unroll
    for (int ty = 0; ty < 2; ++ty)
#pragma unroll
      for (int tx = 0; tx < 3; ++tx) {
        const int hy = ly + ty, hx = lx + tx;
        const int f = ((hx >> 3) ^ (hy & ka.hymask)) & 1;
        a_tab[ty][tx][h] = lds0 + (unsigned)((cfi >> 1) * xpl + (hy * HWc + hx) * 64 + ((((cfi & 1) ^ f)) << 5) + (l15 & 3) * 8);
      }
#pragma unroll
    for (int nf = 0; nf < NF; ++nf) {
      const int nfg = wn * NF + nf;
      const int fd = (p0 >> 3) & 1;
      b_tab[nf][h] = lds0 + (unsigned)(CPT * xpl + (nfg >> 1) * 8192 + p0 * 64 + ((((nfg & 1) ^ fd)) << 5) + (l15 & 3) * 8);
    }
  }
  const unsigned row2 = (unsigned)(2 * HWc * 64);

  f32x4 acc[NTAP][NF];
#pragma unroll
  for (int t = 0; t < NTAP; ++t)
#pragma unroll
    for (int nf = 0; nf < NF; ++nf) acc[t][nf] = (f32x4){0.f, 0.f, 0.f, 0.f};

  auto patch_origin = [&](int patch, int& b, int& oy0, int& ox0) {
    const int q1 = dTX.div(patch);
    const int tx = patch - q1 * ka.tilesX;
    b = dTY.div(q1);
    const int ty = q1 - b * ka.tilesY;
    oy0 = ty * TH; ox0 = tx * TW;
  };
  const uint32_t zlo = (uint32_t)(uintptr_t)ka.zero, zhi = (uint32_t)((uint64_t)(uintptr_t)ka.zero >> 32);
  int nvalid = 0;
#pragma unroll
  for (int c = 0; c < CPT; ++c) nvalid += cvalid[c] ? 1 : 0;
  int dma_cnt = 2 * NPL;
#pragma unroll
  for (int it = 0; it < XIT; ++it) dma_cnt += (it * 256 + wave * 64 < ka.HPv * 4) ? nvalid : 0;
  dma_cnt = __builtin_amdgcn_readfirstlane(dma_cnt);
  auto issue_loads = [&](int patch, int stg) {
    int b, oy0, ox0;
    patch_origin(patch, b, oy0, ox0);
#pragma unroll
    for (int it = 0; it < XIT; ++it) {
      const int v = it * 256 + tid;
      const int R = v >> 2, s = v & 3;
      const int hy = dHW.div(R), hx = R - hy * HWc;
      const int iy = oy0 - 1 + hy, ix = ox0 - 1 + hx;
      const bool inr = v < ka.HPv * 4;
      const bool ok = inr && (unsigned)iy < (unsigned)d.Hin && (unsigned)ix < (unsigned)d.Win;
      const int f = ((hx >> 3) ^ (hy & ka.hymask)) & 1;
      const uint32_t pix = (!SUB || d.in_sy == 0) ? (uint32_t)((b * d.Hin + iy) * d.Win + ix)
                                                  : (uint32_t)((b * d.in_H + (iy * d.in_sy + d.in_oy)) * d.in_W + (ix * d.in_sx + d.in_ox));
      const int sgr = s ^ (f << 1);
      const uint32_t slb = (uint32_t)(sgr * 16);
      if (it * 256 + wave * 64 < ka.HPv * 4) {
#pragma unroll
        for (int c = 0; c < CPT; ++c) {
          if (!cvalid[c]) continue;
          const bool okc = PART ? (ok && sgr * 8 < klen[c]) : ok;
          const uint64_t av = (uint64_t)(uintptr_t)sp[c] + (uint64_t)(pix * cb[c] + slb);
          const uint32_t lo = okc ? (uint32_t)av : zlo, hi = okc ? (uint32_t)(av >> 32) : zhi;
          if (inr) glds16_flat((const unsigned char*)(uintptr_t)(((uint64_t)hi << 32) | lo),
                               lds0 + (unsigned)(stg * stage + c * xpl + (it * 256 + wave * 64) * 16));
        }
      }
    }
#pragma unroll
    for (int it = 0; it < 2; ++it) {
      const int v = it * 256 + tid;
      const int p = v >> 2, s = v & 3;
      const int ly = dTW.div(p), lx = p - ly * TW;
      const bool pv = p < P && oy0 + ly < d.Hout && ox0 + lx < d.Wout;
      const uint32_t pix = (uint32_t)((b * d.Hout + oy0 + ly) * d.Wout + ox0 + lx);
      const int sl = s ^ (((p >> 3) & 1) << 1);
#pragma unroll
      for (int j = 0; j < NPL; ++j) {
        const int n = n0 + j * 32 + sl * 8;
        const bool okn = pv && n < d.N;
        const uint64_t av = (uint64_t)(uintptr_t)dyp + (uint64_t)(pix * dycb + (uint32_t)(n * 2));
        const uint32_t lo = okn ? (uint32_t)av : zlo, hi = okn ? (uint32_t)(av >> 32) : zhi;
        glds16_flat((const unsigned char*)(uintptr_t)(((uint64_t)hi << 32) | lo),
                    lds0 + (unsigned)(stg * stage + CPT * xpl + j * 8192 + (it * 256 + wave * 64) * 16));
      }
    }
  };
  auto transform = [&](int patch, int stg) {
    int b, oy0, ox0;
    patch_origin(patch, b, oy0, ox0);
    unsigned char* const sb = smem + stg * stage;
    const int sl = tid & 3;
#pragma unroll
    for (int c = 0; c < CPT; ++c) {
      if (!cvalid[c]) continue;
      float sc[8], sh[8];
#pragma unroll
      for (int j = 0; j < 8; ++j) { sc[j] = aff_tab[(c * 32 + sl * 8 + j) * 2]; sh[j] = aff_tab[(c * 32 + sl * 8 + j) * 2 + 1]; }
#pragma unroll
      for (int it = 0; it < XIT; ++it) {
        const int v = it * 256 + tid;
        const int R = v >> 2;
        const int hy = dHW.div(R), hx = R - hy * HWc;
        const int iy = oy0 - 1 + hy, ix = ox0 - 1 + hx;
        if (v < ka.HPv * 4 && (unsigned)iy < (unsigned)d.Hin && (unsigned)ix < (unsigned)d.Win) {
          const int f = ((hx >> 3) ^ (hy & ka.hymask)) & 1;
          u32x4* q = (u32x4*)(sb + c * xpl + R * 64 + ((sl ^ (f << 1)) * 16));
          float x[8];
          vec_unpack<T>(*q, x);
#pragma unroll
          for (int j = 0; j < 8; ++j) {
            x[j] = x[j] * sc[j] + sh[j];
            if (aff_relu) x[j] = fmaxf(x[j], 0.f);
          }
          *q = vec_pack<T>(x);
        }
      }
    }
  };

  const int p_begin = split * ka.pps;
  const int p_end = min(ka.patches, p_begin + ka.pps);
  const int npat = p_end - p_begin;
  const int NST = ka.nst;
  const bool mine = cvalid[cfi >> 1];
  __syncthreads();
  for (int j = 0; j < NST - 1 && j < npat; ++j) issue_loads(p_begin + j, j);
  int stg = 0;
  for (int i = 0; i < npat; ++i) {
    const int patch = p_begin + i;
    const int ahead = min(NST - 2, npat - 1 - i);
    vm_wait(ahead * dma_cnt);
    lds_barrier();
    if (i + NST - 1 < npat) issue_loads(patch + NST - 1, stg == 0 ? NST - 1 : stg - 1);
    if constexpr (AFF) {
      transform(patch, stg);
      lds_barrier();
    }
    const unsigned so = (unsigned)(stg * stage);
    stg = stg + 1 == NST ? 0 : stg + 1;
    if (!mine) continue;
    constexpr int AD = !DEEP ? 1 : NF >= 4 ? 4 : (NF == 2 ? 6 : 9);
    auto a_frag = [&](int q) {
      const int ks = q / NTAP, t = q % NTAP, ty = SUB ? R0 + t / 2 : t / 3, tx = SUB ? C0 + t % 2 : t % 3;
      const unsigned o = so + (unsigned)(ks * ka.kstride) + (ty == 2 ? row2 : 0u);
      return tr_frag(a_tab[ty & 1][tx][0] + o, a_tab[ty & 1][tx][1] + o);
    };
    u32x4 af[AD], bf[2][NF];
#pragma unroll
    for (int nf = 0; nf < NF; ++nf) bf[0][nf] = tr_frag(b_tab[nf][0] + so, b_tab[nf][1] + so);
#pragma unroll
    for (int q = 0; q < AD; ++q) af[q] = a_frag(q);
    if constexpr (DEEP) __builtin_amdgcn_sched_barrier(0);
#pragma unroll
    for (int ks = 0; ks < 4; ++ks) {
#pragma unroll
      for (int t = 0; t < NTAP; ++t) {
        const int q = ks * NTAP + t;
        if (t == NTAP / 2 && ks + 1 < 4) {
          const unsigned bo = so + (unsigned)((ks + 1) * 2048);
#pragma unroll
          for (int nf = 0; nf < NF; ++nf) bf[(ks + 1) & 1][nf] = tr_frag(b_tab[nf][0] + bo, b_tab[nf][1] + bo);
        }
#pragma unroll
        for (int nf = 0; nf < NF; ++nf) mma16<T>(acc[t][nf], af[q % AD], bf[ks & 1][nf]);
        if (q + AD < 4 * NTAP) af[q % AD] = a_frag(q + AD);
        if constexpr (DEEP) __builtin_amdgcn_sched_barrier(0);
      }
    }
  }
  if (!mine) return;
  const int Npad = (d.N + 15) & ~15;
  const int Ktot = d.nchunks * 32;
  const int krow0 = (kt * CPT + (cfi >> 1)) * 32 + (cfi & 1) * 16 + g * 4;
#pragma unroll
  for (int t = 0; t < NTAP; ++t)
#pragma unroll
    for (int nf = 0; nf < NF; ++nf) {
      const int n = n0 + (wn * NF + nf) * 16 + l15;
      if (n >= Npad) continue;
#pragma unroll
// ... 57 lines not shown
  g->r0 = g->c0 = -1;
  if (k2) {
    if (!k2_on || d->stride != 1 || (unsigned)d->pad > 1u || !d->pad_x_set || (unsigned)d->pad_x > 1u || !d->use_tap_off || d->src[0].scale) return false;
    g->r0 = 1 - d->pad; g->c0 = 1 - d->pad_x;
  } else if (d->KH != 3 || d->KW != 3 || d->stride != 1 || d->pad != 1 || (d->pad_x_set && d->pad_x != 1) || d->in_sy != 0 || d->use_tap_off) return false;
  if (d->Hin != d->Hout || d->Win != d->Wout || d->N < 1) return false;
  if (((d->N % 8) != 0 || d->N < 16) && (!partial_on_n() || k2 || (d->dyC % 8) || (d->dy_c_off % 8) || d->dy_c_off + ((d->N + 7) & ~7) > d->dyC)) return false;
  static const bool partial_on = (ksmi_knob_int("KSMI_WGRAD3_PARTIAL", 1) != 0);
  for (int i = 0; i < d->nsrc; ++i) {
    if (d->src[i].c_len < 1 || (d->src[i].C % 8) || (d->src[i].c_off % 8) || d->src[i].c_off + ((d->src[i].c_len + 7) & ~7) > d->src[i].C) return false;
    if ((d->src[i].c_len % 32) && (!partial_on || k2)) return false;
    if (d->src[i].scale && (i > 0 || d->nsrc != 1)) return false;
    const size_t ipx = d->in_sy ? (size_t)d->B * d->in_H * d->in_W : (size_t)d->B * d->Hin * d->Win;
    if (ipx * (size_t)d->src[i].C * 2 >= ((size_t)1 << 32)) return false;
  }
  if ((size_t)d->B * d->Hout * d->Wout * (size_t)d->dyC * 2 >= ((size_t)1 << 32)) return false;
  if (d->uniform_kc) { if (d->uniform_kc != 32 || d->k_total > d->nchunks * 32 || d->k_total <= (d->nchunks - 1) * 32) return false; }
  else for (int i = 0; i < d->nchunks; ++i) if (d->k_len[i] < 1 || d->k_len[i] > 32 || (d->k_len[i] != 32 && (!partial_on || k2))) return false;
  const int H = d->Hout, W = d->Wout;
  long best = -1;
  for (int tw = 8; tw <= 32; tw *= 2) {
    const int thmax = 128 / tw;
    const int tilesX = (W + tw - 1) / tw;
    const int tilesY0 = (H + thmax - 1) / thmax;
    const int th = (H + tilesY0 - 1) / tilesY0;
    const int hwc = (tw < W ? tw : W) + 2;
    const long key = (long)tilesX * tilesY0 * 100000 + (long)(thmax + 2) * hwc;
    if ((thmax + 2) * hwc > 256) continue;
    if (best < 0 || key <= best) { best = key;
      g->TW = tw; g->TH = th; g->HWc = hwc; g->tilesX = tilesX; g->tilesY = tilesY0; }
  }
  if (best < 0) return false;
  const int npad = (d->N + 15) & ~15;
  g->WC = d->nchunks == 1 ? 2 : 4;
  g->NTL = npad >= 48 ? 64 : 32;
  if (k2 && (g->WC != 4 || g->NTL != 64)) return false;
  g->KT = (d->nchunks + g->WC / 2 - 1) / (g->WC / 2);
  g->NTt = (npad + g->NTL - 1) / g->NTL;
  g->patches = d->B * g->tilesX * g->tilesY;
  const int hh_alloc = 128 / g->TW + 2;
  g->xpl = hh_alloc * g->HWc * 64;
  g->stage = (g->WC / 2) * g->xpl + (g->NTL / 32) * 8192;
  if (2 * (size_t)g->stage + 1024 > 160 * 1024) return false;
  const int nst_knob = ksmi_knob_int("KSMI_WGRAD3_NST", 2);
  const int nst_want = nst_knob >= 2 ? nst_knob : 2;
  int nst_max = (int)((160 * 1024 - 1024) / g->stage);
  if (nst_max > 4) nst_max = 4;
  if (nst_want < nst_max) nst_max = nst_want;
  const int wg_force = ksmi_knob_int("KSMI_WGRAD3_WGS", 0);
  const int tiles = g->KT * g->NTt;
  const int nfw = (g->NTL / 16) / (4 / g->WC);
  const double ntaps = k2 ? 4.0 : 9.0;
  const double t_patch = 4.0 * ntaps * nfw * 16.0 / 2100.0;
  const double tile_mb = ntaps * (g->WC * 16) * g->NTL * 4.0 / 1e6;
  const double op_bytes = (double)d->B * H * W * (d->nchunks * 32.0 + npad) * 2.0;
  const size_t lds2 = 2 * (size_t)g->stage + 1024;
  const int max_per_cu = (int)(160 * 1024 / lds2) < 4 ? (int)(160 * 1024 / lds2) : 4;
  static const double eff[5] = {0.0, 0.35, 0.8, 0.85, 0.9};
  double best_t = 1e30;
  static const int cand[] = {128, 192, 256, 384, 512, 768, 1024};
  for (int ci = 0; ci < 7; ++ci) {
    const int wg = wg_force ? wg_force : cand[ci];
    if (wg > 256 * max_per_cu && !wg_force) break;
    int want = wg / tiles;
    if (want < 1) want = 1;
    if (want > g->patches) want = g->patches;
    const int pps = (g->patches + want - 1) / want;
    const int ns = (g->patches + pps - 1) / pps;
    int per_cu = (ns * tiles + 255) / 256;
    if (per_cu > 4) per_cu = 4;
    const int nst = per_cu == 1 ? nst_max : 2;
    const double e = eff[per_cu];
    double t_main = pps * t_patch * per_cu / e;
    double bw = (double)ns * tiles * g->stage / 5.0;
    if (bw > 4.5e6) bw = 4.5e6;
    if (t_main < op_bytes / bw) t_main = op_bytes / bw;
    const double t = t_main + 7.0 + 2.0 * ns * tiles * tile_mb / 4.0;
    if (t < best_t) { best_t = t; g->pps = pps; g->nsplit = ns; g->nst = nst; }
  }
  g->lds = (size_t)g->nst * g->stage + 1024;
  return true;
}

int ksmi_wgrad3_reduce(const ksmi_wgrad_desc* d, const ksmi_wgrad3_geom_t* g, hipStream_t st) {
  const int ntaps = g->r0 >= 0 ? 4 : 9;
  const size_t total4 = (size_t)ntaps * d->nchunks * 32 * ((d->N + 15) & ~15) / 4;
  hipLaunchKernelGGL(wgrad3_reduce_kernel, dim3((unsigned)((total4 + 15) / 16)), dim3(256), 0, st, *d, g->nsplit, ntaps);
  return ksmi_check_launch("wgrad3_reduce");
}

int ksmi_wgrad3_launch(const ksmi_wgrad_desc* d, const ksmi_wgrad3_geom_t* g, hipStream_t st) {
  Wg3Args ka;
  ka.d = *d;
  ka.TH = g->TH; ka.TW = g->TW; ka.HWc = g->HWc; ka.HPv = (g->TH + 2) * g->HWc;
  ka.xpl = g->xpl; ka.stage = g->stage;
  ka.tilesX = g->tilesX; ka.tilesY = g->tilesY; ka.patches = g->patches; ka.pps = g->pps;
  ka.KT = g->KT; ka.NTt = g->NTt;
  ka.m_hw = fastdiv_magic(g->HWc); ka.m_tw = fastdiv_magic(g->TW); ka.m_tx = fastdiv_magic(g->tilesX); ka.m_ty = fastdiv_magic(g->tilesY);
  ka.m_tiles = fastdiv_magic(g->KT * g->NTt); ka.m_ntt = fastdiv_magic(g->NTt);
  ka.kstride = (32 / g->TW) * g->HWc * 64;
  ka.hymask = g->TW == 8 ? 1 : 0;
  ka.lds_bytes = (int)g->lds;
  ka.nst = g->nst;
  const unsigned char* const zero_page = wg3_zero();
  if (!zero_page) return ksmi_fail(KSMI_E_UNSUPPORTED, "wgrad3: zero page");
  ka.zero = zero_page;
  if ((size_t)g->patches * 1 >= ((size_t)1 << 31) / 1024) return ksmi_fail(KSMI_E_UNSUPPORTED, "wgrad3: too many patches");
  const dim3 grid(g->nsplit * g->KT * g->NTt);
  const bool aff = d->src[0].scale != nullptr;
  static const bool deep = (ksmi_knob_int("KSMI_WGRAD3_DEEP", 1) != 0);
#define KSMI_W3_(WC_, WN_, NF_, AFF_, DEEP_)                                                          \
  do {                                                                                               \
    auto kfn = wgrad3_kernel<WC_, WN_, NF_, AFF_, DEEP_>; KSMI_NOTE(kfn);                            \
    if (g->lds > 65536) (void)hipFuncSetAttribute((const void*)kfn, hipFuncAttributeMaxDynamicSharedMemorySize, (int)g->lds); \
    hipLaunchKernelGGL(kfn, grid, dim3(256), g->lds, st, ka);                                        \
  } while (0)
#define KSMI_W3(WC_, WN_, NF_)                                                                       \
  do {                                                                                               \
    if (aff) { if (deep) KSMI_W3_(WC_, WN_, NF_, true, true); else KSMI_W3_(WC_, WN_, NF_, true, false); }   \
    else { if (deep) KSMI_W3_(WC_, WN_, NF_, false, true); else KSMI_W3_(WC_, WN_, NF_, false, false); }     \
  } while (0)
  if (g->r0 >= 0) {
#define KSMI_W3K(R0_, C0_)                                                                           \
  do {                                                                                               \
    auto kfn = wgrad3_kernel<4, 1, 4, false, true, R0_, C0_>; KSMI_NOTE(kfn);                        \
    if (g->lds > 65536) (void)hipFuncSetAttribute((const void*)kfn, hipFuncAttributeMaxDynamicSharedMemorySize, (int)g->lds); \
    hipLaunchKernelGGL(kfn, grid, dim3(256), g->lds, st, ka);                                        \
  } while (0)
    if (aff || g->WC != 4 || g->NTL != 64) return ksmi_fail(KSMI_E_UNSUPPORTED, "wgrad3: no 2 x 2 instance");
    if (g->r0 == 0 && g->c0 == 0) KSMI_W3K(0, 0); else if (g->r0 == 0) KSMI_W3K(0, 1); else if (g->c0 == 0) KSMI_W3K(1, 0); else KSMI_W3K(1, 1);
#undef KSMI_W3K
    return ksmi_check_launch("wgrad3");
  }
  bool part = false;
  for (int i = 0; i < d->nsrc; ++i) part = part || (d->src[i].c_len % 32) != 0;
  if (part) {
#define KSMI_W3P(WC_, WN_, NF_)                                                                      \
  do {                                                                                               \
    if (aff) { auto kfn = wgrad3_kernel<WC_, WN_, NF_, true, true, -1, -1, true>; KSMI_NOTE(kfn);    \
      if (g->lds > 65536) (void)hipFuncSetAttribute((const void*)kfn, hipFuncAttributeMaxDynamicSharedMemorySize, (int)g->lds); \
      hipLaunchKernelGGL(kfn, grid, dim3(256), g->lds, st, ka); }                                    \
    else { auto kfn = wgrad3_kernel<WC_, WN_, NF_, false, true, -1, -1, true>; KSMI_NOTE(kfn);       \
      if (g->lds > 65536) (void)hipFuncSetAttribute((const void*)kfn, hipFuncAttributeMaxDynamicSharedMemorySize, (int)g->lds); \
      hipLaunchKernelGGL(kfn, grid, dim3(256), g->lds, st, ka); }                                    \
  } while (0)
    if (g->WC == 4 && g->NTL == 64) KSMI_W3P(4, 1, 4);
    else if (g->WC == 4) KSMI_W3P(4, 1, 2);
    else if (g->NTL == 64) KSMI_W3P(2, 2, 2);
    else KSMI_W3P(2, 2, 1);
#undef KSMI_W3P
    return ksmi_check_launch("wgrad3");
  }
  if (g->WC == 4 && g->NTL == 64) KSMI_W3(4, 1, 4);
  else if (g->WC == 4) KSMI_W3(4, 1, 2);
  else if (g->NTL == 64) KSMI_W3(2, 2, 2);
  else KSMI_W3(2, 2, 1);
#undef KSMI_W3
#undef KSMI_W3_
  return ksmi_check_launch("wgrad3");
}
```

### kurosiwo_amd/functional.py

```python
import ctypes as C

import torch

from . import _lib
from .runtime import DT, SrcSpec, conv_grid_m, conv_npad, conv_stats_rows, make_conv, make_pack, make_wgrad, packed_weight_numel, require_gpu, stream_ptr


def to_nhwc(x_nchw, dtype):
    require_gpu(x_nchw)
    B, Cc, H, W = x_nchw.shape
    y = torch.empty((B, H, W, Cc), dtype=dtype, device=x_nchw.device)
    _lib.check(_lib.load().ksmi_nchw_to_nhwc(x_nchw.contiguous().float().data_ptr(), y.data_ptr(), B, Cc, H * W, DT[dtype], stream_ptr()))
    return y


def to_nchw(x_nhwc):
    B, H, W, Cc = x_nhwc.shape
    y = torch.empty((B, Cc, H, W), dtype=torch.float32, device=x_nhwc.device)
    _lib.check(_lib.load().ksmi_nhwc_to_nchw(x_nhwc.data_ptr(), y.data_ptr(), B, Cc, H * W, DT[x_nhwc.dtype], stream_ptr()))
    return y


def _pack(weight, table, taps, N, n_mod, sK, sN, sD, sT, flip, dtype):
    Npad = conv_npad(N)
    out = torch.empty(packed_weight_numel(table, taps, Npad, dtype), dtype=dtype, device=weight.device)
    d = make_pack(weight, out, table, taps, N, Npad, n_mod, sK, sN, sD, sT, flip)
    _lib.check(_lib.load().ksmi_pack_weights(C.byref(d), DT[dtype], stream_ptr()), "pack_weights")
    return out


def conv3x3(xs, weight, bias=None, affine=None, want_stats=False, alpha=0.0, relu_out=0, resid=None, mask=None, out=None, accumulate=0,
            gate=None):
    dtype = xs[0].dtype
    B, H, W, _ = xs[0].shape
    N = weight.shape[0]
    Ktot = sum(x.shape[3] for x in xs)
    srcs = [SrcSpec(x, x.shape[3]) for x in xs]
    if affine is not None:
        srcs[0].scale, srcs[0].shift, srcs[0].relu = affine
    if out is None:
        out = torch.empty((B, H, W, N), dtype=dtype, device=xs[0].device)
    d, table = make_conv(srcs, [(out, out.shape[3], 0, 0, N, accumulate)], out, bias, None, B, H, W, H, W, 3, 3, 1, 1, N, dtype,
                         alpha=alpha, relu_out=relu_out, resid=None if resid is None else (resid, resid.shape[3]), mask=mask)
    wpk = _pack(weight.contiguous(), table, 9, N, N, 9, Ktot * 9, 0, 1, 0, dtype)
    d.wpk = wpk.data_ptr()
    if gate is not None:
        d.gate_src, d.xhat_src, d.g_mean, d.g_rstd = (t.data_ptr() for t in gate)
        if not _lib.load().ksmi_conv_gate_supported(C.byref(d), DT[dtype]):
            raise _lib.KsmiError("conv3x3: the gate epilogue is not available for this shape")
    stats = None
    if want_stats:
        stats = torch.zeros((conv_stats_rows(d, dtype), 2, d.Npad), dtype=torch.float32, device=out.device)
        d.stats = stats.data_ptr()
    _lib.check(_lib.load().ksmi_conv_forward(C.byref(d), DT[dtype], stream_ptr()), "conv_forward")
    return out, stats


def conv3x3_dgrad(dy, weight, splits):
    dtype = dy.dtype
    B, H, W, N = dy.shape
    Ktot = sum(splits)
    outs = [torch.empty((B, H, W, c), dtype=dtype, device=dy.device) for c in splits]
    dsts, nb = [], 0
    for o, c in zip(outs, splits):
        dsts.append((o, c, 0, nb, c, 0))
        nb += c
    d, table = make_conv([SrcSpec(dy, N)], dsts, dy, None, None, B, H, W, H, W, 3, 3, 1, 1, Ktot, dtype)
    wpk = _pack(weight.contiguous(), table, 9, Ktot, Ktot, Ktot * 9, 9, 0, 1, 1, dtype)
    d.wpk = wpk.data_ptr()
    _lib.check(_lib.load().ksmi_conv_forward(C.byref(d), DT[dtype], stream_ptr()), "conv_dgrad")
    return outs


def conv3x3_wgrad(xs, dy, affine=None, n_real=None):
    dtype = dy.dtype
    B, H, W, dyC = dy.shape
    N = dyC if n_real is None else n_real
    Ktot = sum(x.shape[3] for x in xs)
    srcs = [SrcSpec(x, x.shape[3]) for x in xs]
    if affine is not None:
        srcs[0].scale, srcs[0].shift, srcs[0].relu = affine
    grad = torch.zeros((N, Ktot, 3, 3), dtype=torch.float32, device=dy.device)
    d, ws = make_wgrad(srcs, dy, dyC, 0, N, grad, 9, Ktot * 9, 1, 0, B, H, W, H, W, 3, 3, 1, 1, dtype)
    wsb = torch.empty(max(ws, 16), dtype=torch.uint8, device=dy.device)
    d.partial = wsb.data_ptr()
    _lib.check(_lib.load().ksmi_conv_wgrad(C.byref(d), DT[dtype], stream_ptr()), "conv_wgrad")
    return grad


def deconv2x2(x, weight, bias):
    dtype = x.dtype
    B, H, W, Cin = x.shape
    Cout = weight.shape[1]
    y = torch.empty((B, 2 * H, 2 * W, Cout), dtype=dtype, device=x.device)
    d, table = make_conv([SrcSpec(x, Cin)], [(y, Cout, 0, 0, 4 * Cout, 0)], x, bias, None, B, H, W, H, W, 1, 1, 1, 0,
                         4 * Cout, dtype, ps_cout=Cout)
    wpk = _pack(weight.contiguous(), table, 1, 4 * Cout, Cout, Cout * 4, 4, 1, 0, 0, dtype)
    d.wpk = wpk.data_ptr()
    _lib.check(_lib.load().ksmi_conv_forward(C.byref(d), DT[dtype], stream_ptr()), "deconv_forward")
    return y


def deconv2x2_backward(x, dy, weight):
    dtype = x.dtype
    B, H, W, Cin = x.shape
    Cout = weight.shape[1]
    dx = torch.empty_like(x)
    s2 = [SrcSpec(dy, Cout)]
    d2, t2 = make_conv(s2, [(dx, Cin, 0, 0, Cin, 0)], dy, None, None, B, 2 * H, 2 * W, H, W, 2, 2, 2, 0, Cin, dtype)
    w2 = _pack(weight.contiguous(), t2, 4, Cin, Cin, 4, Cout * 4, 0, 1, 0, dtype)
    d2.wpk = w2.data_ptr()
    _lib.check(_lib.load().ksmi_conv_forward(C.byref(d2), DT[dtype], stream_ptr()), "deconv_dgrad")
    grad = torch.zeros_like(weight)
    dw, ws = make_wgrad(s2, x, Cin, 0, Cin, grad, 4, Cout * 4, 1, 0, B, 2 * H, 2 * W, H, W, 2, 2, 2, 0, dtype)
    wsb = torch.empty(max(ws, 16), dtype=torch.uint8, device=x.device)
    dw.partial = wsb.data_ptr()
    _lib.check(_lib.load().ksmi_conv_wgrad(C.byref(dw), DT[dtype], stream_ptr()), "deconv_wgrad")
    return dx, grad


def linear(x, weight, bias=None, out=None, accumulate=0):
    dtype = x.dtype
    rows, Cin = x.shape
    N = weight.shape[0]
    if out is None:
        out = torch.empty((rows, N), dtype=dtype, device=x.device)
    d, table = make_conv([SrcSpec(x, Cin)], [(out, N, 0, 0, N, accumulate)], out, bias, None, 1, rows, 1, rows, 1, 1, 1, 1, 0, N, dtype)
    wpk = _pack(weight.contiguous(), table, 1, N, N, 1, Cin, 0, 0, 0, dtype)
    d.wpk = wpk.data_ptr()
    _lib.check(_lib.load().ksmi_conv_forward(C.byref(d), DT[dtype], stream_ptr()), "linear")
    return out


def linear_dgrad(dy, weight, out=None, accumulate=0):
    dtype = dy.dtype
    rows, N = dy.shape
    Cin = weight.shape[1]
    if out is None:
        out = torch.empty((rows, Cin), dtype=dtype, device=dy.device)
    d, table = make_conv([SrcSpec(dy, N)], [(out, Cin, 0, 0, Cin, accumulate)], out, None, None, 1, rows, 1, rows, 1, 1, 1, 1, 0, Cin, dtype)
    wpk = _pack(weight.contiguous(), table, 1, Cin, Cin, Cin, 1, 0, 0, 0, dtype)
    d.wpk = wpk.data_ptr()
    _lib.check(_lib.load().ksmi_conv_forward(C.byref(d), DT[dtype], stream_ptr()), "linear_dgrad")
    return out


def linear_wgrad(x, dy, with_bias=False):
    dtype = x.dtype
    rows, Cin = x.shape
    N = dy.shape[1]
    grad = torch.zeros((N, Cin), dtype=torch.float32, device=x.device)
    d, ws = make_wgrad([SrcSpec(x, Cin)], dy, N, 0, N, grad, 1, Cin, 0, 0, 1, rows, 1, rows, 1, 1, 1, 1, 0, dtype)
    wsb = torch.empty(max(ws, 16), dtype=torch.uint8, device=x.device)
    d.partial = wsb.data_ptr()
    lib = _lib.load()
    mode, bias_buf = 0, None
    if with_bias:
        bias_buf = torch.full((max(d.nsplit, 1), N), float("nan"), dtype=torch.float32, device=x.device)
        d.bias_grad = bias_buf.data_ptr()
        mode = int(lib.ksmi_conv_wgrad_fuses_bias(C.byref(d), DT[dtype]))
        if mode == 0:
            d.bias_grad = None
    _lib.check(lib.ksmi_conv_wgrad(C.byref(d), DT[dtype], stream_ptr()), "linear_wgrad")
    if not with_bias:
        return grad
    db = None if mode == 0 else (bias_buf[0].clone() if mode == 1 else bias_buf[:d.nsplit].sum(0))
    return grad, db, mode


def layernorm(x, gamma, beta, eps=1e-5):
# ... 182 lines not shown
```

### kurosiwo_amd/runtime.py

```python
import ctypes as C
import functools

import torch

from . import _lib
from ._lib import KSMI_BF16, KSMI_F32, ConvDesc, Dst, PackDesc, Src, WgradDesc, check

DT = {torch.float32: KSMI_F32, torch.bfloat16: KSMI_BF16}


def require_gpu(t):
    if not t.is_cuda:
        raise _lib.KsmiError("kurosiwo_amd runs on an MI355X (HIP) device only: got a CPU tensor. "
                             "There is no CPU fallback; use the reference repo for CPU runs.")


def stream_ptr():
    return C.c_void_p(torch.cuda.current_stream().cuda_stream)


def ptr(t):
    return C.c_void_p(t.data_ptr()) if t is not None else C.c_void_p(0)


# ... 167 lines not shown
    _fill_srcs(d, srcs)
    d.ndst = len(dsts)
    for i, (t, Cc, c_off, nb, nl, acc) in enumerate(dsts):
        q = d.dst[i]
        q.ptr, q.C, q.c_off, q.n_begin, q.n_len, q.accumulate = t.data_ptr(), Cc, c_off, nb, nl, acc
    d.wpk = wpk.data_ptr()
    d.bias = bias.data_ptr() if bias is not None else None
    d.stats = stats.data_ptr() if stats is not None else None
    if mask is not None:
        d.mask_src, d.m_mean, d.m_rstd, d.m_scale, d.m_shift = [x.data_ptr() for x in mask]
    d.B, d.Hin, d.Win, d.Hout, d.Wout = B, Hin, Win, Hout, Wout
    d.KH, d.KW, d.stride, d.pad = KH, KW, stride, pad
    d.pad_x = pad if pad_x is None else pad_x
    if in_map is not None:
        d.in_sy, d.in_sx, d.in_oy, d.in_ox, d.in_H, d.in_W = in_map
    d.alpha, d.relu_out = alpha, relu_out
    if resid is not None:
        d.resid, d.residC = resid[0].data_ptr(), resid[1]
    if out_map is not None:
        d.out_sy, d.out_sx, d.out_oy, d.out_ox, d.out_H, d.out_W = out_map
    mp = max_pix if stride == 1 else min(max_pix, 128)
    d.TH, d.TW = choose_patch(Hout, Wout, stride, KH, KW, mp)
    d.N, d.Npad = N, conv_npad(N)
    d.nchunks = len(table)
    d.ps_cout = ps_cout
    if _uniform(table, kc)[0]:
        d.uniform_kc = kc
    else:
        for i, (si, c0, _, _) in enumerate(table):
            d.chunk_src[i], d.chunk_c0[i] = si, c0
    return d, table


def conv_grid_m(d):
    return _lib.load().ksmi_conv_grid_m(C.byref(d))


def conv_stats_rows(d, dtype):
    import os
    if os.environ.get("KSMI_STATS_ROWS_TILE") == "1":
        return conv_grid_m(d)
    rows = _lib.load().ksmi_conv_stats_rows(C.byref(d), DT[dtype])
    d.stats_rows = rows
    return rows


def packed_weight_numel(table, taps, Npad, dtype):
    return len(table) * taps * Npad * chunk_elems(dtype)


def make_wgrad(srcs, dy, dyC, dy_c_off, N, grad, gK, gN, gT, accumulate, B, Hin, Win, Hout, Wout,
               KH, KW, stride, pad, dtype, pad_x=None, in_map=None, tap_off=None):
    kc = chunk_elems(dtype)
    table, _ = _chunk_table(srcs, kc)
    d = WgradDesc()
    _fill_srcs(d, srcs)
    d.dy, d.dyC, d.dy_c_off = dy.data_ptr(), dyC, dy_c_off
    d.B, d.Hin, d.Win, d.Hout, d.Wout = B, Hin, Win, Hout, Wout
    d.KH, d.KW, d.stride, d.pad = KH, KW, stride, pad
    mp = 256 if stride == 1 else 128
    d.TH, d.TW = choose_patch_wgrad(Hout, Wout, stride, KH, KW, mp)
    d.N, d.nchunks = N, len(table)
    if pad_x is not None:
        d.pad_x_set, d.pad_x = 1, pad_x
    if in_map is not None:
        d.in_sy, d.in_sx, d.in_oy, d.in_ox, d.in_H, d.in_W = in_map
    if tap_off is not None:
        d.use_tap_off = 1
        for i, t in enumerate(tap_off):
            d.tap_off[i] = t
    d.grad, d.gK, d.gN, d.gT, d.accumulate = grad.data_ptr(), gK, gN, gT, accumulate
    kc_u, ktot = _uniform(table, kc)
    if kc_u:
        d.uniform_kc, d.k_total = kc_u, ktot
    else:
        for i, (si, c0, kg, kl) in enumerate(table):
            d.chunk_src[i], d.chunk_c0[i], d.k_off[i], d.k_len[i] = si, c0, kg, kl
    lib = _lib.load()
    ws = lib.ksmi_conv_wgrad_workspace(C.byref(d), DT[dtype])
    npad = (N + 15) // 16 * 16
    slab = (KH * KW) * len(table) * kc * npad * 4
    d.nsplit = ws // slab
    return d, ws
```

### kurosiwo_amd/snunet_plan.py

```python
import ctypes as C
import os

import torch

from . import _lib
from .plan_base import PlanBase, _Saved
from .runtime import Act, SrcSpec, conv_npad, conv_stats_rows, make_conv, make_pack, make_wgrad, packed_weight_numel
from .snunet import BN_EPS, BN_MOMENTUM


class SNUNetPlan(PlanBase):
    side_wgrad = True
    two_lanes = True
    bn_fused = os.environ.get("KSMI_BN_FUSED", "1") != "0"
    im2col_late = os.environ.get("KSMI_IM2COL_LATE", "1") != "0"
    up_gemm = os.environ.get("KSMI_UP_GEMM", "1") != "0"
    up_wgrad64 = os.environ.get("KSMI_UP_WGRAD64", "1") != "0"
    up_wgrad128 = os.environ.get("KSMI_UP_WGRAD128", "1") != "0"
    pack_kind = "pack_weights_batched"

    def __init__(self, model, B, H, W, dtype, training, with_backward, tail=0, sync_bn=False):
        self._init_lists(model, dtype, with_backward)
        self.B, self.H, self.W = B, H, W
        from . import distributed as _D
        self.sync_bn = bool(sync_bn) and training
        self.bn_world = _D.world_size() if self.sync_bn else 1
        if self.sync_bn:
            self.bn_fused = False
        self.training = training
        self._up_packs = []
        self._rowsums = []
        n, c = model.base_channel, model.in_channels
        self.n = n
        f = [n, 2 * n, 4 * n, 8 * n, 16 * n]
        self.tail = tail
        self.xA = torch.empty((B, c - tail, H, W), dtype=torch.float32, device=self.dev)
        self.xB = torch.empty_like(self.xA)
        self.xtail = torch.empty((B, tail, H, W), dtype=torch.float32, device=self.dev) if tail else None
        self.logits = torch.empty((B, 3, H, W), dtype=torch.float32, device=self.dev)
        self.dlogits = torch.empty_like(self.logits) if with_backward else None
        self.bwd_builders = []

        def A(name, lvl, ch):
            return Act(name, B, H >> lvl, W >> lvl, ch, dtype, self.dev)

        L = self._lane
        L(0); x0_0A, p0A = self._block("conv0_0", "A", [self.xA], A("x0_0A", 0, f[0]), first=True, pool="p0A")
        self._handover(0, 1, back=(1, 0))
        L(1); x0_0B, p0B = self._block("conv0_0", "B", [self.xB], A("x0_0B", 0, f[0]), first=True, pool="p0B")
        L(0); x1_0A, p1A = self._block("conv1_0", "A", [self._pool_at(x0_0A, p0A, "p0A")], A("x1_0A", 1, f[1]), pool="p1A")
        self._handover(0, 1, back=(1, 0))
        L(1); x1_0B, p1B = self._block("conv1_0", "B", [self._pool_at(x0_0B, p0B, "p0B")], A("x1_0B", 1, f[1]), pool="p1B")
        L(0); x2_0A, p2A = self._block("conv2_0", "A", [self._pool_at(x1_0A, p1A, "p1A")], A("x2_0A", 2, f[2]), pool="p2A")
        self._handover(0, 1, back=(1, 0))
        L(1); x2_0B, p2B = self._block("conv2_0", "B", [self._pool_at(x1_0B, p1B, "p1B")], A("x2_0B", 2, f[2]), pool="p2B")
        L(0); x3_0A = self._block("conv3_0", "A", [self._pool_at(x2_0A, p2A, "p2A")], A("x3_0A", 3, f[3]))
        self._handover(0, 1, back=(1, 0))
        L(1); x3_0B, p3B = self._block("conv3_0", "B", [self._pool_at(x2_0B, p2B, "p2B")], A("x3_0B", 3, f[3]), pool="p3B")
        x4_0B = self._block("conv4_0", "B", [self._pool_at(x3_0B, p3B, "p3B")], A("x4_0B", 4, f[4]))
        self._handover(1, 0, back=(0, 1))

        self._handover(0, 1, back=(1, 0))
        L(0); x0_1 = self._block("conv0_1", "", [x0_0A, x0_0B, self._up("Up1_0", x1_0B)], A("x0_1", 0, f[0]))
        L(1); x1_1 = self._block("conv1_1", "", [x1_0A, x1_0B, self._up("Up2_0", x2_0B)], A("x1_1", 1, f[1]))
        u1_1 = self._up("Up1_1", x1_1)
        self._handover(1, 0, back=(0, 1))
        L(0); x0_2 = self._block("conv0_2", "", [x0_0A, x0_0B, x0_1, u1_1], A("x0_2", 0, f[0]))
        L(1); x2_1 = self._block("conv2_1", "", [x2_0A, x2_0B, self._up("Up3_0", x3_0B)], A("x2_1", 2, f[2]))
        x1_2 = self._block("conv1_2", "", [x1_0A, x1_0B, x1_1, self._up("Up2_1", x2_1)], A("x1_2", 1, f[1]))
        u1_2 = self._up("Up1_2", x1_2)
        self._handover(1, 0, back=(0, 1))
        L(0); x0_3 = self._block("conv0_3", "", [x0_0A, x0_0B, x0_1, x0_2, u1_2], A("x0_3", 0, f[0]))
        L(1); x3_1 = self._block("conv3_1", "", [x3_0A, x3_0B, self._up("Up4_0", x4_0B)], A("x3_1", 3, f[3]))
        x2_2 = self._block("conv2_2", "", [x2_0A, x2_0B, x2_1, self._up("Up3_1", x3_1)], A("x2_2", 2, f[2]))
        x1_3 = self._block("conv1_3", "", [x1_0A, x1_0B, x1_1, x1_2, self._up("Up2_2", x2_2)], A("x1_3", 1, f[1]))
        u1_3 = self._up("Up1_3", x1_3)
        self._handover(1, 0, back=(0, 1))
        L(0); x0_4 = self._block("conv0_4", "", [x0_0A, x0_0B, x0_1, x0_2, x0_3, u1_3], A("x0_4", 0, f[0]))
        self._head([x0_1, x0_2, x0_3, x0_4])
        self.acts = {a.name: a for a in (x0_0A, x0_0B, x1_0A, x1_0B, x3_0B, x4_0B, x0_1, x1_1, x0_2, x0_3, x0_4, x1_3, x3_1)}

        if with_backward:
            for lane, build in reversed(self.bwd_builders):
                self._lane(lane)
                build()
            self._lane(0)
        self._finish()

    def _before_pack_table(self):
        if self._rowsums:
            nr = len(self._rowsums)
            arr_r = (_lib.RowsumDesc * nr)(*[r for r, _ in self._rowsums])
            raw_r = bytes(C.string_at(C.addressof(arr_r), C.sizeof(arr_r)))
            rtable = torch.frombuffer(bytearray(raw_r), dtype=torch.uint8).to(self.dev)
            self.keep.append(rtable)
            self.bwd.add("ksmi_reduce_rows_batched", lambda: (rtable.data_ptr(), nr))
            self._mark(*[k for _, k in self._rowsums])
        for i in range(0, len(self._up_packs), 16):
            grp = self._up_packs[i:i + 16]
            wt_a = (C.c_void_p * len(grp))(*[w.data_ptr() for w, _, _ in grp])
            wb_a = (C.c_void_p * len(grp))(*[b.data_ptr() for _, b, _ in grp])
            c_a = (C.c_int * len(grp))(*[c for _, _, c in grp])
            self.keep += [wt_a, wb_a, c_a]
            self.packs.add("ksmi_up_pack_weights_batched", lambda wt_a=wt_a, wb_a=wb_a, c_a=c_a, k=len(grp): (wt_a, wb_a, c_a, k),
                           {"kind": "up_pack_weight", "bytes": sum(4 * c * c * 6 for _, _, c in grp), "flops": 0})

    def _lane(self, lane):
        self.fwd.cur_lane = self.bwd.cur_lane = lane

    def _level(self, H):
        lvl = {self.H >> k: k for k in range(5)}.get(H)
        self._stage(None if lvl is None else f"L{lvl}")

    def _sname(self, name):
        return name if self.fwd.cur_lane == 0 else f"{name}@{self.fwd.cur_lane}"

    def _handover(self, src, dst, back):
        self.fwd.add_wait(src, dst)
        a, b = back
        self.bwd_builders.append((0, lambda: self.bwd.add_wait(a, b)))

    def _rows(self, npix):
        return max(1, min(512, npix // 256))

    def _rowsum_at_end(self, key, partial, rows, K, k, Cstride, Cc):
        r = _lib.RowsumDesc()
        r.partial = partial.data_ptr() if partial is not None else None
        r.dst = self.m._g(key).data_ptr()
        r.rows, r.K, r.k, r.Cstride, r.C = (rows if partial is not None else 0), K, k, Cstride, Cc
        r.accumulate, r.head, r.next = 0, 1, -1
        if self._acc_param(key):
            prev = [q for q, kk in self._rowsums if kk == key][-1]
            prev.next, r.head = len(self._rowsums), 0
        if partial is not None:
            self.keep.append(partial)
        self._rowsums.append((r, key))

    def _conv(self, ll, d, tag="fwd", name=""):
        self.keep.append(d)
        meta, ktot, _ = self._conv_meta(d, tag, f",BN{32 if d.Npad >= 32 else 16}")
        meta["tag"] = f"K={ktot} N={d.N} {d.Hout}x{d.Wout} nsrc={d.nsrc}"
        ll.add("ksmi_conv_forward", lambda: (C.byref(d), self.dt), meta)

    def _side_ix(self, key):
        if os.environ.get("KSMI_SIDE2", "0") != "1":
            return 0
        if not hasattr(self, "_side_of"):
            self._side_of = {}
        if key not in self._side_of:
            self._side_of[key] = len(self._side_of) & 1
        return self._side_of[key]

    def _wgrad(self, d, ws, key, side_tag=None):
        assert side_tag is None
        self.keep.append(d)
        six = self._side_ix(key)
        sW = self._sname("wgrad" + ("_s2" if six else ""))
        self.need(sW, ws)
        self.patch(d, "partial", sW)
        meta, ktot, _ = self._wgrad_meta(d)
        meta["tag"] = f"{key} K={ktot} N={d.N} {d.Hout}x{d.Wout}"
        meta["side"] = True
        meta["side_ix"] = six
        self.bwd.add("ksmi_conv_wgrad", lambda: (C.byref(d), self.dt), meta)
        self._mark(key)

    def _emit_dgrad(self, act, bias_key=None, gate=None):
        cons = getattr(act, "consumers", [])
        if not cons:
            return False
        B, H, W, Cc = act.B, act.H, act.W, act.C
        srcs = [SrcSpec(r, cj) for (r, cj, _, _, _) in cons]
        acc = act.take_acc_flag()
        d, table = make_conv(srcs, [(act.grad(), Cc, 0, 0, Cc, acc)], act.grad(), None, None, B, H, W, H, W, 3, 3, 1, 1, Cc, self.dtype)
        Npad = conv_npad(Cc)
        wpk = torch.empty(packed_weight_numel(table, 9, Npad, self.dtype), dtype=self.dtype, device=self.dev)
        kc = 32 if self.dtype == torch.bfloat16 else 16
        slab = 9 * Npad * kc
        ch0 = 0
        for (r, cj, wkey, coff, ktot) in cons:
            nch = -(-cj // kc)
            tj = [(0, c0, c0, min(kc, cj - c0)) for c0 in range(0, cj, kc)]
            wview = self.m._p(wkey)[coff * 9:]
            out = wpk[ch0 * slab:(ch0 + nch) * slab]
            pd = make_pack(wview, out, tj, 9, Cc, Npad, Cc, ktot * 9, 9, 0, 1, 1)
            self.keep += [pd, wview, out]
            self._pack_descs.append(pd)
            ch0 += nch
        d.wpk = wpk.data_ptr()
        self.keep.append(wpk)
        gated = None
        if gate is not None:
            g_out, g_z, g_sv = gate
            d.gate_src, d.xhat_src, d.g_mean, d.g_rstd = g_out.data_ptr(), g_z.data_ptr(), g_sv.mean, g_sv.rstd
            if self.lib.ksmi_conv_gate_supported(C.byref(d), self.dt):
                rows_g = conv_stats_rows(d, self.dtype)
                st = torch.empty(rows_g * 2 * Npad, dtype=torch.float32, device=self.dev)
                d.stats = st.data_ptr()
                self.keep.append(st)
                gated = (st, rows_g, Npad)
            else:
                d.gate_src = d.xhat_src = d.g_mean = d.g_rstd = None
        if bias_key is not None:
            rows_g = conv_stats_rows(d, self.dtype)
            st = torch.empty(rows_g * 2 * Npad, dtype=torch.float32, device=self.dev)
            d.stats = st.data_ptr()
            self._rowsum_at_end(bias_key, st, rows_g, 2, 0, Npad, Cc)
        self._conv(self.bwd, d, "dgrad")
        return gated if gated is not None else True

    def _pool(self, x, name):
        y = Act(name, x.B, x.H // 2, x.W // 2, x.C, self.dtype, self.dev)
        self._level(x.H)
        self.fwd.add("ksmi_maxpool2x2_forward", lambda: (x.t.data_ptr(), y.t.data_ptr(), x.B, x.H, x.W, x.C, self.dt))
        self._pool_bwd(x, y)
        return y

    def _pool_at(self, x, y, name):
        if y is None:
            return self._pool(x, name)
        self._pool_bwd(x, y)
        return y

    def _pool_bwd(self, x, y):
        def build_bwd():
            self._level(x.H)
            self._emit_dgrad(y)
            acc = x.take_acc_flag()
            gy, gx = y.grad(), x.grad()
            self.bwd.add("ksmi_maxpool2x2_backward", lambda: (x.t.data_ptr(), gy.data_ptr(), gx.data_ptr(), acc,
                                                              x.B, x.H, x.W, x.C, self.dt))
        self.bwd_builders.append((self.fwd.cur_lane, build_bwd))

    def _up_conv_forward(self, x, y, wkey, bkey, B, H, W, Cc):
        d, table = make_conv([SrcSpec(x.t, Cc)], [(y.t, Cc, 0, 0, 4 * Cc, 0)], x.t, self.m._p(bkey), None,
                             B, H, W, H, W, 1, 1, 1, 0, 4 * Cc, self.dtype, ps_cout=Cc)
        wpk = self._packed(wkey, table, 1, 4 * Cc, Cc, Cc * 4, 4, 1, 0, 0)
        d.wpk = wpk.data_ptr()
        self._conv(self.fwd, d)

    def _up(self, name, x):
        Cc, B, H, W = x.C, x.B, x.H, x.W
        y = Act(name, B, 2 * H, 2 * W, Cc, self.dtype, self.dev)
        self._level(2 * H)
        wkey, bkey = f"{name}.up.weight", f"{name}.up.bias"
        up_gemm = (self.up_gemm and self.dtype == torch.bfloat16 and bool(self.lib.ksmi_up_gemm_supported(B, H, W, Cc, self.dt)))
        up_fwd_gemm = up_gemm and Cc >= 256
        up_wgrad_gemm = up_fwd_gemm or (self.up_gemm and ((self.up_wgrad64 and Cc == 64) or (self.up_wgrad128 and Cc == 128))
                                        and self.dtype == torch.bfloat16 and bool(self.lib.ksmi_up_wgrad_supported(B, H, W, Cc, self.dt)))
        es = self._es()
        if up_gemm:
            wb = torch.empty(4 * Cc * Cc, dtype=torch.bfloat16, device=self.dev)
            self.keep.append(wb)
            self._up_packs.append((self.m._p(wkey), wb, Cc))
        if up_fwd_gemm:
            self.fwd.add("ksmi_up_forward", lambda: (x.t.data_ptr(), wb.data_ptr(), self.m._p(bkey).data_ptr(), y.t.data_ptr(), B, H, W, Cc),
                         {"kind": "up_gemm_fwd", "bytes": B * H * W * Cc * 5 * es, "flops": 2 * B * H * W * Cc * 4 * Cc, "tag": f"K={Cc} N={4 * Cc} {H}x{W}"})
        else:
            self._up_conv_forward(x, y, wkey, bkey, B, H, W, Cc)

        def build_bwd():
            self._level(2 * H)
            fused_bias = self._emit_dgrad(y, bias_key=bkey)
            gy = y.grad()
            s2 = [SrcSpec(gy, Cc)]
            acc = x.take_acc_flag()
            if up_gemm:
                gx = x.grad()
                self.bwd.add("ksmi_up_dgrad", lambda: (gy.data_ptr(), wb.data_ptr(), gx.data_ptr(), acc, B, H, W, Cc),
                             {"kind": "up_gemm_dgrad", "bytes": B * H * W * Cc * (5 + acc) * es, "flops": 2 * B * H * W * Cc * 4 * Cc,
                              "tag": f"K={4 * Cc} N={Cc} {H}x{W}"})
            else:
                d2, t2 = make_conv(s2, [(x.grad(), Cc, 0, 0, Cc, acc)], gy, None, None,
                                   B, 2 * H, 2 * W, H, W, 2, 2, 2, 0, Cc, self.dtype)
                w2 = self._packed(wkey, t2, 4, Cc, Cc, 4, Cc * 4, 0, 1, 0)
                d2.wpk = w2.data_ptr()
                self._conv(self.bwd, d2, "dgrad")
            if up_wgrad_gemm:
                six = self._side_ix(wkey)
                sW = self._sname("wgrad" + ("_s2" if six else ""))
                self.need(sW, self.lib.ksmi_up_wgrad_workspace(B, H, W, Cc))
                a_w = self._acc_param(wkey)
                self.bwd.add("ksmi_up_wgrad", lambda: (x.t.data_ptr(), gy.data_ptr(), self.scr(sW), self.m._g(wkey).data_ptr(), a_w, B, H, W, Cc),
                             {"kind": "up_gemm_wgrad", "bytes": B * H * W * Cc * 5 * es + 16 * Cc * Cc, "flops": 2 * B * H * W * Cc * 4 * Cc,
                              "tag": f"{wkey} K={Cc} N={4 * Cc} {H}x{W}", "side": True, "side_ix": six})
                self._mark(wkey)
            else:
                dw, ws = make_wgrad(s2, x.t, Cc, 0, Cc, self.m._g(wkey), 4, Cc * 4, 1, self._acc_param(wkey),
                                    B, 2 * H, 2 * W, H, W, 2, 2, 2, 0, self.dtype)
                self._wgrad(dw, ws, wkey)
            if not fused_bias:
                npix = B * 4 * H * W
                rows = self._rows(npix)
                pb = torch.empty(rows * Cc, dtype=torch.float32, device=self.dev)
                self.bwd.add("ksmi_channel_sum", lambda: (gy.data_ptr(), pb.data_ptr(), rows, npix, Cc, self.dt))
                self._rowsum_at_end(bkey, pb, rows, 1, 0, Cc, Cc)
        self.bwd_builders.append((self.fwd.cur_lane, build_bwd))
        return y

    def _block(self, name, branch, sources, out, first=False, pool=None):
        m, B, H, W, Cc = self.m, out.B, out.H, out.W, out.C
        npix = B * H * W
        dtype, dt, training = self.dtype, self.dt, self.training
        self._level(H)
        i_act = Act(f"{name}{branch}.i", B, H, W, Cc, dtype, self.dev)
        z_act = Act(f"{name}{branch}.z", B, H, W, Cc, dtype, self.dev)
        sv1, sv2 = _Saved(Cc, self.dev), _Saved(Cc, self.dev)
        self.keep += [i_act, z_act, sv1, sv2]
        P = lambda s: m._p(f"{name}.{s}").data_ptr()
        G = lambda s: m._g(f"{name}.{s}").data_ptr()
        Bf = lambda s: m._b(f"{name}.{s}").data_ptr()
        Npad = conv_npad(Cc)
        sS, sR = self._sname("stats"), self._sname("red")
        stats = (lambda: self.scr(sS)) if training else (lambda: None)

        if first:
            x_img = sources[0]
            chead, cin = x_img.shape[1], m.in_channels
            x_tail = self.xtail.data_ptr() if self.tail else None
            kc = 32 if dtype == torch.bfloat16 else 16
            Kpad = -(-(cin * 9) // kc) * kc
            rows1, cpad1, Ktot = self.lib.ksmi_conv_first_stats_rows(B, H, W), Cc, cin
            self.need(sS, rows1 * 2 * Cc * 4)
            raw = m._raw_ptrs(self.dev)
            self.fwd.add("ksmi_conv_first_forward_raw", lambda: (x_img.data_ptr(), x_tail, chead, P("conv1.weight"), P("conv1.bias"),
                                                                 i_act.t.data_ptr(), stats(), B, cin, H, W, Cc, *raw, dt))
            if self.with_backward:
                col = torch.empty((B, H, W, Kpad), dtype=dtype, device=self.dev)
                self.keep.append(col)
                im2col_args = lambda: (x_img.data_ptr(), x_tail, chead, col.data_ptr(), B, cin, H, W, Kpad, *raw, dt)
                if not self.im2col_late:
                    self.fwd.add("ksmi_im2col3x3_raw", im2col_args)
                src1 = [SrcSpec(col, Kpad)]
        else:
            srcs = [SrcSpec(a.t, a.C) for a in sources]
            Ktot = sum(a.C for a in sources)
            d1, t1 = make_conv(srcs, [(i_act.t, Cc, 0, 0, Cc, 0)], i_act.t, m._p(f"{name}.conv1.bias"), None,
                               B, H, W, H, W, 3, 3, 1, 1, Cc, dtype)
            w1 = self._packed(f"{name}.conv1.weight", t1, 9, Cc, Cc, 9, Ktot * 9, 0, 1, 0)
            d1.wpk = w1.data_ptr()
            rows1, cpad1 = conv_stats_rows(d1, dtype), Npad
            if training:
                self.need(sS, rows1 * 2 * Npad * 4)
                self.patch(d1, "stats", sS)
            self._conv(self.fwd, d1)

        gcount = float(npix * self.bn_world)

        def bn_fin(bn, sv, rows, cpad):
            nbt = m._c(f"{name}.{bn}.num_batches_tracked").data_ptr()
            if self.sync_bn:
                self.fwd.add_allreduce(lambda rows=rows, cpad=cpad: self._bufs[sS][:rows * 2 * cpad * 4].view(torch.float32))
            self.fwd.add("ksmi_bn_finalize", lambda: (stats(), rows, cpad, Cc, gcount, P(f"{bn}.weight"), P(f"{bn}.bias"),
                                                      Bf(f"{bn}.running_mean"), Bf(f"{bn}.running_var"), nbt,
                                                      BN_MOMENTUM, BN_EPS, 1 if training else 0,
                                                      sv.mean, sv.rstd, sv.scale, sv.shift))
        bn_fin("bn1", sv1, rows1, cpad1)

        src2 = [SrcSpec(i_act.t, Cc, scale=sv1.scale_t, shift=sv1.shift_t, relu=1)]
        d2, t2 = make_conv(src2, [(z_act.t, Cc, 0, 0, Cc, 0)], z_act.t, m._p(f"{name}.conv2.bias"), None,
                           B, H, W, H, W, 3, 3, 1, 1, Cc, dtype)
        w2 = self._packed(f"{name}.conv2.weight", t2, 9, Cc, Cc, 9, Cc * 9, 0, 1, 0)
        d2.wpk = w2.data_ptr()
        rows2 = conv_stats_rows(d2, dtype)
        if training:
            self.need(sS, rows2 * 2 * Npad * 4)
            self.patch(d2, "stats", sS)
        self._conv(self.fwd, d2)
        fused = training and self.bn_fused and bool(self.lib.ksmi_bn_fused_supported(Cc, Npad, dt))
        pooled = None
        if fused:
            if pool is not None:
                pooled = Act(pool, B, H // 2, W // 2, Cc, dtype, self.dev)
            nbt2 = m._c(f"{name}.bn2.num_batches_tracked").data_ptr()
            pp = pooled.t.data_ptr() if pooled is not None else None
            self.fwd.add("ksmi_bn_fin_add_relu", lambda: (stats(), rows2, Npad, Cc, float(npix), P("bn2.weight"), P("bn2.bias"),
                                                          Bf("bn2.running_mean"), Bf("bn2.running_var"), nbt2, BN_MOMENTUM, BN_EPS,
                                                          sv2.mean, sv2.rstd, sv2.scale, sv2.shift, z_act.t.data_ptr(), i_act.t.data_ptr(),
                                                          out.t.data_ptr(), pp, B, H, W, dt),
                         {"kind": "bn_fin_add_relu", "bytes": npix * Cc * self._es() * (3.25 if pooled is not None else 3), "flops": 0})
        else:
            bn_fin("bn2", sv2, rows2, Npad)
            self.fwd.add("ksmi_bn_add_relu", lambda: (z_act.t.data_ptr(), i_act.t.data_ptr(), sv2.scale, sv2.shift,
                                                      out.t.data_ptr(), npix, Cc, dt))

        def build_bwd():
            self._level(H)
            gated = self._emit_dgrad(out, gate=(out.t, z_act.t, sv2)) if os.environ.get("KSMI_NO_GATE") is None else self._emit_dgrad(out)
            gated = gated if isinstance(gated, tuple) else None
            rows = self._rows(npix)
            self.need(sR, rows * 2 * Cc * 4)
            sums1 = torch.zeros((2, Cc), dtype=torch.float32, device=self.dev)
            sums2 = torch.zeros((2, Cc), dtype=torch.float32, device=self.dev)
            dz = torch.empty_like(z_act.t)
            r = torch.empty_like(i_act.t)
            self.keep += [sums1, sums2, dz, r]
            gout = out.grad().data_ptr()
            s1p, s2p = sums1.data_ptr(), sums2.data_ptr()
            a_bn2 = self._acc_param(f"{name}.bn2")
            es = self._es()
            if gated is not None:
                gst, grows, gpad = gated
                if fused and self.lib.ksmi_bn_fused_supported(Cc, gpad, dt):
                    self.bwd.add("ksmi_bn_bwd_fin_apply_gated", lambda: (gst.data_ptr(), grows, gpad, s2p, G("bn2.weight"), G("bn2.bias"), a_bn2,
                                                                         gout, z_act.t.data_ptr(), sv2.mean, sv2.rstd, P("bn2.weight"),
                                                                         dz.data_ptr(), float(npix), npix, Cc, dt),
                                 {"kind": "bn_bwd_fin_apply_gated", "bytes": npix * Cc * es * 3, "flops": 0})
                    self._mark(f"{name}.bn2.weight", f"{name}.bn2.bias")
                else:
                    self.bwd.add("ksmi_reduce_rows", lambda: (gst.data_ptr(), grows, 2, gpad, Cc, s2p, G("bn2.weight"), G("bn2.bias"), a_bn2))
                    self._mark(f"{name}.bn2.weight", f"{name}.bn2.bias")
                    if self.sync_bn:
                        self.bwd.add_allreduce(lambda: sums2)
                    self.bwd.add("ksmi_bn_bwd_apply_gated", lambda: (gout, z_act.t.data_ptr(), sv2.mean, sv2.rstd, P("bn2.weight"), s2p,
                                                                     dz.data_ptr(), gcount, npix, Cc, dt))
            else:
                self.bwd.add("ksmi_bnrelu_bwd_reduce", lambda: (gout, out.t.data_ptr(), z_act.t.data_ptr(), sv2.mean, sv2.rstd,
                                                                self.scr(sR), rows, npix, Cc, dt))
                if fused:
                    self.bwd.add("ksmi_bnrelu_bwd_fin_apply", lambda: (self.scr(sR), rows, Cc, s2p, G("bn2.weight"), G("bn2.bias"), a_bn2,
                                                                       gout, out.t.data_ptr(), z_act.t.data_ptr(), sv2.mean, sv2.rstd,
                                                                       P("bn2.weight"), dz.data_ptr(), float(npix), npix, Cc, dt),
                                 {"kind": "bnrelu_bwd_fin_apply", "bytes": npix * Cc * es * 5, "flops": 0})
                    self._mark(f"{name}.bn2.weight", f"{name}.bn2.bias")
                else:
                    self.bwd.add("ksmi_reduce_rows", lambda: (self.scr(sR), rows, 2, Cc, Cc, s2p, G("bn2.weight"), G("bn2.bias"), a_bn2))
                    self._mark(f"{name}.bn2.weight", f"{name}.bn2.bias")
                    if self.sync_bn:
                        self.bwd.add_allreduce(lambda: sums2)
                    self.bwd.add("ksmi_bnrelu_bwd_apply", lambda: (gout, out.t.data_ptr(), z_act.t.data_ptr(), sv2.mean, sv2.rstd,
                                                                   P("bn2.weight"), s2p, dz.data_ptr(), gcount, npix, Cc, dt))
            if training:
                self._rowsum_at_end(f"{name}.conv2.bias", None, 0, 1, 0, Cc, Cc)
            else:
                pz = torch.empty(rows * Cc, dtype=torch.float32, device=self.dev)
                self.bwd.add("ksmi_channel_sum", lambda: (dz.data_ptr(), pz.data_ptr(), rows, npix, Cc, dt))
                self._rowsum_at_end(f"{name}.conv2.bias", pz, rows, 1, 0, Cc, Cc)
            dg2, tg2 = make_conv([SrcSpec(dz, Cc)], [(r, Cc, 0, 0, Cc, 0)], dz, None, None, B, H, W, H, W, 3, 3, 1, 1, Cc, dtype,
                                 mask=(i_act.t, sv1.t[0], sv1.t[1], sv1.t[2], sv1.t[3]))
            wg2 = self._packed(f"{name}.conv2.weight", tg2, 9, Cc, Cc, Cc * 9, 9, 0, 1, 1)
            dg2.wpk = wg2.data_ptr()
            rows_g = conv_stats_rows(dg2, dtype)
            self.need(sS, rows_g * 2 * Npad * 4)
            self.patch(dg2, "stats", sS)
            self._conv(self.bwd, dg2, "dgrad")
            a_bn1 = self._acc_param(f"{name}.bn1")
            if not fused:
                self.bwd.add("ksmi_reduce_rows", lambda: (self.scr(sS), rows_g, 2, Npad, Cc, s1p, G("bn1.weight"), G("bn1.bias"), a_bn1))
                self._mark(f"{name}.bn1.weight", f"{name}.bn1.bias")
                if self.sync_bn:
                    self.bwd.add_allreduce(lambda: sums1)
            dw2, ws2 = make_wgrad(src2, dz, Cc, 0, Cc, m._g(f"{name}.conv2.weight"), 9, Cc * 9, 1,
                                  self._acc_param(f"{name}.conv2.weight"), B, H, W, H, W, 3, 3, 1, 1, dtype)
            self._wgrad(dw2, ws2, f"{name}.conv2.weight")
            pb1 = torch.empty(rows * Cc, dtype=torch.float32, device=self.dev)
            if fused:
                rows_b = min(rows, self.lib.ksmi_bn_fused_max_rows())
                self.bwd.add("ksmi_bn_bwd_fin_apply_add", lambda: (self.scr(sS), rows_g, Npad, s1p, G("bn1.weight"), G("bn1.bias"), a_bn1,
                                                                   r.data_ptr(), gout, i_act.t.data_ptr(), sv1.mean, sv1.rstd, P("bn1.weight"),
                                                                   pb1.data_ptr(), rows_b, float(npix), npix, Cc, dt),
                             {"kind": "bn_bwd_fin_apply_add", "bytes": npix * Cc * self._es() * 4, "flops": 0})
                self._mark(f"{name}.bn1.weight", f"{name}.bn1.bias")
                self._rowsum_at_end(f"{name}.conv1.bias", pb1, rows_b, 1, 0, Cc, Cc)
            else:
                self.bwd.add("ksmi_bn_bwd_apply_add", lambda: (r.data_ptr(), gout, i_act.t.data_ptr(), sv1.mean, sv1.rstd,
                                                               P("bn1.weight"), s1p, pb1.data_ptr(), rows, gcount, npix, Cc, dt))
                self._rowsum_at_end(f"{name}.conv1.bias", pb1, rows, 1, 0, Cc, Cc)
            a_w1 = self._acc_param(f"{name}.conv1.weight")
            if first:
                if self.im2col_late:
                    self.bwd.add("ksmi_im2col3x3_raw", im2col_args, {"kind": "im2col3x3_raw", "bytes": B * H * W * (cin * 4 + Kpad * self._es()), "flops": 0})
                dw1, ws1 = make_wgrad(src1, r, Cc, 0, Cc, m._g(f"{name}.conv1.weight"), 1, cin * 9, 0, a_w1,
                                      B, H, W, H, W, 1, 1, 1, 0, dtype)
                for ci in range(dw1.nchunks):
                    dw1.k_len[ci] = max(0, min(dw1.k_len[ci], cin * 9 - dw1.k_off[ci]))
                self._wgrad(dw1, ws1, f"{name}.conv1.weight")
            else:
                srcs = [SrcSpec(a.t, a.C) for a in sources]
                nb = 0
                for a in sources:
                    a.consumers.append((r, Cc, f"{name}.conv1.weight", nb, Ktot))
                    nb += a.C
                dw1, ws1 = make_wgrad(srcs, r, Cc, 0, Cc, m._g(f"{name}.conv1.weight"), 9, Ktot * 9, 1, a_w1,
                                      B, H, W, H, W, 3, 3, 1, 1, dtype)
                self._wgrad(dw1, ws1, f"{name}.conv1.weight")
        self.bwd_builders.append((self.fwd.cur_lane, build_bwd))
        if pool is not None:
            return out, pooled
        return out

    def _head(self, xs):
        m, B, n = self.m, self.B, self.n
        HW = self.H * self.W
        dev, dt = self.dev, self.dt
        self._stage("head")
        f32 = dict(dtype=torch.float32, device=dev)
        avg, mx = torch.zeros((B, 5 * n), **f32), torch.zeros((B, 5 * n), **f32)
        argmax = torch.zeros((B, 5 * n), dtype=torch.int32, device=dev)
        ca, ca1 = torch.zeros((B, 4 * n), **f32), torch.zeros((B, n), **f32)
        hidden = torch.zeros((B, 2, 4 * n // 16 + n // 4), **f32)
        xarr = (C.c_void_p * 4)(*[a.t.data_ptr() for a in xs])
        ws_pool = torch.empty(self.lib.ksmi_ecam_pool_workspace(B, HW, n), dtype=torch.uint8, device=dev)
        self.keep += [avg, mx, argmax, ca, ca1, hidden, xarr, ws_pool]
        self.head = dict(avg=avg, mx=mx, argmax=argmax, ca=ca, ca1=ca1)
        P = lambda key: m._p(key).data_ptr()
        G = lambda key: m._g(key).data_ptr()
        T0 = B * HW * n * self._es()
        self.fwd.add("ksmi_ecam_pool", lambda: (xarr, avg.data_ptr(), mx.data_ptr(), argmax.data_ptr(), ws_pool.data_ptr(), B, HW, n, dt),
                     {"kind": "ecam_pool", "bytes": 4 * T0, "flops": 0})
        self.fwd.add("ksmi_ecam_mlp", lambda: (avg.data_ptr(), mx.data_ptr(), P("ca.fc1.weight"), P("ca.fc2.weight"),
                                               P("ca1.fc1.weight"), P("ca1.fc2.weight"), ca.data_ptr(), ca1.data_ptr(),
                                               hidden.data_ptr(), B, n))
        self.fwd.add("ksmi_ecam_final_forward", lambda: (xarr, ca.data_ptr(), ca1.data_ptr(), P("conv_final.weight"),
                                                         P("conv_final.bias"), self.logits.data_ptr(), B, HW, n, 3, dt),
                     {"kind": "ecam_final_forward", "bytes": 4 * T0 + B * HW * 3 * 4, "flops": 2 * B * HW * 4 * n * 3})

        def build_bwd():
            self._stage("head")
            dca, dca1 = torch.zeros((B, 4 * n), **f32), torch.zeros((B, n), **f32)
            davg, dmax = torch.zeros((B, 5 * n), **f32), torch.zeros((B, 5 * n), **f32)
            ws_b = torch.empty(self.lib.ksmi_ecam_bwd_workspace(B, HW, n, 3), dtype=torch.uint8, device=dev)
            ws_m = torch.empty(self.lib.ksmi_ecam_mlp_bwd_workspace(B, n), dtype=torch.uint8, device=dev)
            garr = (C.c_void_p * 4)(*[a.grad().data_ptr() for a in xs])
            for a in xs:
                a.take_acc_flag()
            for key in ("conv_final.weight", "conv_final.bias", "ca.fc1.weight", "ca.fc2.weight", "ca1.fc1.weight", "ca1.fc2.weight"):
                self._acc_param(key)
            self.keep += [dca, dca1, davg, dmax, ws_b, ws_m, garr]
            dl = self.dlogits.data_ptr()
            self.bwd.add("ksmi_ecam_final_backward_reduce", lambda: (
                xarr, dl, ca.data_ptr(), ca1.data_ptr(), P("conv_final.weight"), dca.data_ptr(), dca1.data_ptr(),
                G("conv_final.weight"), G("conv_final.bias"), ws_b.data_ptr(), B, HW, n, 3, dt),
                {"kind": "ecam_final_backward_reduce", "bytes": 4 * T0 + B * HW * 3 * 4, "flops": 2 * B * HW * 4 * n * 3})
            self._mark("conv_final.weight", "conv_final.bias")
            self.bwd.add("ksmi_ecam_mlp_backward", lambda: (
                avg.data_ptr(), mx.data_ptr(), hidden.data_ptr(), ca.data_ptr(), ca1.data_ptr(), dca.data_ptr(), dca1.data_ptr(),
                P("ca.fc1.weight"), P("ca.fc2.weight"), P("ca1.fc1.weight"), P("ca1.fc2.weight"), davg.data_ptr(), dmax.data_ptr(),
                G("ca.fc1.weight"), G("ca.fc2.weight"), G("ca1.fc1.weight"), G("ca1.fc2.weight"), ws_m.data_ptr(), B, n))
            self._mark("ca.fc1.weight", "ca.fc2.weight", "ca1.fc1.weight", "ca1.fc2.weight")
            self.bwd.add("ksmi_ecam_final_backward_dx", lambda: (
                garr, dl, ca.data_ptr(), P("conv_final.weight"), davg.data_ptr(), dmax.data_ptr(), argmax.data_ptr(), B, HW, n, 3, dt),
                {"kind": "ecam_final_backward_dx", "bytes": 4 * T0 + B * HW * 3 * 4, "flops": 2 * B * HW * 4 * n * 3})
        self.bwd_builders.append((self.fwd.cur_lane, build_bwd))

    def run_forward(self, xA, xB, tail=None):
        if (tail is None) != (self.xtail is None):
            raise _lib.KsmiError("plan and call disagree about the shared tail channels (DEM)")
        return self._run_forward(self.logits, (xA, self.xA), (xB, self.xB), *([] if tail is None else [(tail, self.xtail)]))
```

Baseline: 2298 tiles/s.

## Fuse Siamese encoder weight-gradient convs of both branches into one two-segment wgrad

Adds a DUAL variant of the wgrad3 kernel. It treats the two Siamese branches (A and B) as one batch of 2B, switching the source pointer, dy pointer and BN affine table by batch index. The plan defers branch B's wgrad and emits a single launch when branch A arrives, which removes the separate accumulate pass and gives each launch more work. The first conv also drops im2col in favour of a compact NHWC padded input, so its wgrad can use the 3x3 dual path. The cost is more template instances and deferred scheduling that ties the two branches' backward together, which may reduce overlap across streams.

```diff
diff --git a/include/ksmi.h b/include/ksmi.h
--- a/include/ksmi.h
+++ b/include/ksmi.h
@@ -132,10 +132,13 @@
   int32_t use_tap_off;
   int32_t tap_off[16];
   float* bias_grad; int32_t bias_accumulate;
+  int32_t seg_B;
+  const void* seg_ptr; const void* seg_dy; const float* seg_scale; const float* seg_shift;
 } ksmi_wgrad_desc;
 size_t ksmi_conv_wgrad_workspace(const ksmi_wgrad_desc* d, int dtype);
 int ksmi_conv_wgrad(const ksmi_wgrad_desc* d, int dtype, void* stream);
 int ksmi_conv_wgrad_fuses_bias(const ksmi_wgrad_desc* d, int dtype);
+int ksmi_conv_wgrad_dual_supported(const ksmi_wgrad_desc* d, int dtype);
 
 int ksmi_conv_first_forward(const float* x_nchw, const float* w, const float* bias, void* out, float* stats,
                             int B, int Cin, int H, int W, int Cout, int dtype, void* stream);
@@ -146,6 +149,8 @@
 int ksmi_im2col3x3(const float* x_nchw, void* out, int B, int Cin, int H, int W, int Kpad, int dtype, void* stream);
 int ksmi_im2col3x3_raw(const float* x_nchw, const float* x_tail, int c_head, void* out, int B, int Cin, int H, int W,
                        int Kpad, const float* mean, const float* stdv, const float* clamp, int dtype, void* stream);
+int ksmi_first_nhwc_raw(const float* x_nchw, const float* x_tail, int c_head, void* out, int B, int Cin, int H, int W,
+                        int Cpad, const float* mean, const float* stdv, const float* clamp, int dtype, void* stream);
 int ksmi_conv_first_wgrad(const float* x_nchw, const void* dy, float* dw, float* workspace, size_t ws_bytes,
                           int B, int Cin, int H, int W, int Cout, int accumulate, int dtype, void* stream);
 size_t ksmi_conv_first_wgrad_workspace(int B, int Cin, int H, int W, int Cout);
diff --git a/kurosiwo_amd/_lib.py b/kurosiwo_amd/_lib.py
--- a/kurosiwo_amd/_lib.py
+++ b/kurosiwo_amd/_lib.py
@@ -76,7 +76,8 @@
                 ("uniform_kc", C.c_int32), ("k_total", C.c_int32),
                 ("in_sy", C.c_int32), ("in_sx", C.c_int32), ("in_oy", C.c_int32), ("in_ox", C.c_int32), ("in_H", C.c_int32), ("in_W", C.c_int32),
                 ("pad_x_set", C.c_int32), ("pad_x", C.c_int32), ("use_tap_off", C.c_int32), ("tap_off", C.c_int32 * 16),
-                ("bias_grad", C.c_void_p), ("bias_accumulate", C.c_int32)]
+                ("bias_grad", C.c_void_p), ("bias_accumulate", C.c_int32),
+                ("seg_B", C.c_int32), ("seg_ptr", C.c_void_p), ("seg_dy", C.c_void_p), ("seg_scale", C.c_void_p), ("seg_shift", C.c_void_p)]
 
 
 class Op(C.Structure):
@@ -109,6 +110,7 @@
     "ksmi_conv_wgrad_workspace": (_sz, [C.POINTER(WgradDesc), _i]),
     "ksmi_conv_wgrad": (_i, [C.POINTER(WgradDesc), _i, _vp]),
     "ksmi_conv_wgrad_fuses_bias": (_i, [C.POINTER(WgradDesc), _i]),
+    "ksmi_conv_wgrad_dual_supported": (_i, [C.POINTER(WgradDesc), _i]),
     "ksmi_conv_stats_rows": (_i, [C.POINTER(ConvDesc), _i]),
     "ksmi_conv_gate_supported": (_i, [C.POINTER(ConvDesc), _i]),
     "ksmi_desc_size": (C.c_size_t, [_i]),
@@ -117,6 +119,7 @@
     "ksmi_conv_first_stats_rows": (_i, [_i, _i, _i]),
     "ksmi_im2col3x3": (_i, [_vp, _vp, _i, _i, _i, _i, _i, _i, _vp]),
     "ksmi_im2col3x3_raw": (_i, [_vp, _vp, _i, _vp, _i, _i, _i, _i, _i, _vp, _vp, _vp, _i, _vp]),
+    "ksmi_first_nhwc_raw": (_i, [_vp, _vp, _i, _vp, _i, _i, _i, _i, _i, _vp, _vp, _vp, _i, _vp]),
     "ksmi_conv_first_wgrad": (_i, [_vp, _vp, _vp, _vp, _sz, _i, _i, _i, _i, _i, _i, _i, _vp]),
     "ksmi_conv_first_wgrad_workspace": (_sz, [_i, _i, _i, _i, _i]),
     "ksmi_bn_finalize": (_i, [_vp, _i, _i, _i, _d, _vp, _vp, _vp, _vp, _vp, _f, _f, _i, _vp, _vp, _vp, _vp, _vp]),
diff --git a/kurosiwo_amd/csrc/elementwise.hip b/kurosiwo_amd/csrc/elementwise.hip
--- a/kurosiwo_amd/csrc/elementwise.hip
+++ b/kurosiwo_amd/csrc/elementwise.hip
@@ -556,6 +556,28 @@
       f[j] = c < Cin ? xs[c * 324 + (ly + t / 3) * 18 + lx + t % 3] : 0.f;
     }
     *(u32x4*)(out + (((int64_t)b * H + oy) * W + ox) * Kpad + q * VEC) = vec_pack<T>(f);
+  }
+}
+
+template <typename T>
+__global__ __launch_bounds__(256) void first_nhwc_kernel(const float* __restrict__ x, T* out, int B, int Cin, int H, int W, int Cpad,
+                                                         const float* __restrict__ nmean, const float* __restrict__ nstd,
+                                                         const float* __restrict__ nclamp, const float* __restrict__ xtail, int chead) {
+  constexpr int VEC = ElemTraits<T>::kVec;
+  const int64_t npix = (int64_t)B * H * W;
+  for (int64_t p = (int64_t)blockIdx.x * 256 + threadIdx.x; p < npix; p += (int64_t)gridDim.x * 256) {
+    const int ix = (int)(p % W);
+    const int64_t q = p / W;
+    const int iy = (int)(q % H), b = (int)(q / H);
+    for (int c0 = 0; c0 < Cpad; c0 += VEC) {
+      float f[VEC];
+#pragma unroll
+      for (int j = 0; j < VEC; ++j) {
+        const int c = c0 + j;
+        f[j] = c < Cin ? raw_tile_value(image_value(x, xtail, chead, Cin, b, c, H, W, iy, ix), c, nmean, nstd, nclamp) : 0.f;
+      }
+      *(u32x4*)(out + p * Cpad + c0) = vec_pack<T>(f);
+    }
   }
 }
 
@@ -1040,6 +1062,18 @@
   return ksmi_check_launch("im2col3x3");
 }
 
+int ksmi_first_nhwc_raw(const float* x_nchw, const float* xtail, int chead, void* out, int B, int Cin, int H, int W, int Cpad,
+                        const float* nmean, const float* nstd, const float* nclamp, int dtype, void* stream) {
+  if (int rc = first_conv_sources(xtail, &chead, Cin, nmean, nstd, nclamp)) return rc;
+  if (!x_nchw || !out || B < 1 || H < 1 || W < 1 || Cin < 1 || Cin > 32 || Cpad != ((Cin + 7) & ~7))
+    return ksmi_fail(KSMI_E_ARG, "first_nhwc: need 1 <= Cin <= 32 and Cpad = Cin rounded up to 8");
+  const int grid = grid_for((int64_t)B * H * W, 8192);
+  KSMI_DT(dtype,
+          hipLaunchKernelGGL(first_nhwc_kernel<bf16_t>, dim3(grid), dim3(256), 0, (hipStream_t)stream, x_nchw, (bf16_t*)out, B, Cin, H, W, Cpad, nmean, nstd, nclamp, xtail, chead),
+          hipLaunchKernelGGL(first_nhwc_kernel<float>, dim3(grid), dim3(256), 0, (hipStream_t)stream, x_nchw, (float*)out, B, Cin, H, W, Cpad, nmean, nstd, nclamp, xtail, chead));
+  return ksmi_check_launch("first_nhwc");
+}
+
 int ksmi_im2col3x3(const float* x_nchw, void* out, int B, int Cin, int H, int W, int Kpad, int dtype, void* stream) {
   return ksmi_im2col3x3_raw(x_nchw, nullptr, Cin, out, B, Cin, H, W, Kpad, nullptr, nullptr, nullptr, dtype, stream);
 }
diff --git a/kurosiwo_amd/csrc/igemm.hip b/kurosiwo_amd/csrc/igemm.hip
--- a/kurosiwo_amd/csrc/igemm.hip
+++ b/kurosiwo_amd/csrc/igemm.hip
@@ -796,6 +796,8 @@
   WgradGeom g = wgrad_geom<T>(d);
   if (d->TH * d->TW > 256) return ksmi_fail(KSMI_E_ARG, "wgrad: patch too large");
   if (d->nsplit != g.nsplit) return ksmi_fail(KSMI_E_ARG, "wgrad: nsplit does not match ksmi_conv_wgrad_workspace geometry");
+  if (d->seg_B != 0 && !(g.v3 && ksmi_wgrad3_dual_ok(d, &g.g3)))
+    return ksmi_fail(KSMI_E_UNSUPPORTED, "wgrad: no two-segment kernel for this descriptor (ksmi_conv_wgrad_dual_supported)");
   if (g.v3) {
     int rc3 = ksmi_wgrad3_launch(d, &g.g3, st);
     if (rc3) return rc3;
@@ -1017,6 +1019,12 @@
   return wgrad_slab_bias_on() && (g.tbt == 64 || g.tbt == 96 || g.tbt == 128) ? 2 : 0;
 }
 
+int ksmi_conv_wgrad_dual_supported(const ksmi_wgrad_desc* d, int dtype) {
+  if (!d || dtype != KSMI_BF16 || d->nsrc != 1 || d->nchunks < 1) return 0;
+  WgradGeom g = wgrad_geom<bf16_t>(d);
+  return g.v3 && ksmi_wgrad3_dual_ok(d, &g.g3) ? 1 : 0;
+}
+
 int ksmi_conv_wgrad(const ksmi_wgrad_desc* d, int dtype, void* stream) {
   if (!d || d->nsrc < 1 || d->nsrc > KSMI_MAX_SRC || d->nchunks < 1 || (d->nchunks > KSMI_MAX_CHUNKS && !(d->uniform_kc && d->nsrc == 1)))
     return ksmi_fail(KSMI_E_ARG, "wgrad: bad descriptor");
diff --git a/kurosiwo_amd/csrc/wgrad3.h b/kurosiwo_amd/csrc/wgrad3.h
--- a/kurosiwo_amd/csrc/wgrad3.h
+++ b/kurosiwo_amd/csrc/wgrad3.h
@@ -13,5 +13,6 @@
   size_t lds;
 };
 bool ksmi_wgrad3_geom(const ksmi_wgrad_desc* d, int dtype, ksmi_wgrad3_geom_t* g);
+bool ksmi_wgrad3_dual_ok(const ksmi_wgrad_desc* d, const ksmi_wgrad3_geom_t* g);
 int ksmi_wgrad3_launch(const ksmi_wgrad_desc* d, const ksmi_wgrad3_geom_t* g, hipStream_t st);
 int ksmi_wgrad3_reduce(const ksmi_wgrad_desc* d, const ksmi_wgrad3_geom_t* g, hipStream_t st);
diff --git a/kurosiwo_amd/csrc/wgrad3.hip b/kurosiwo_amd/csrc/wgrad3.hip
--- a/kurosiwo_amd/csrc/wgrad3.hip
+++ b/kurosiwo_amd/csrc/wgrad3.hip
@@ -41,7 +41,7 @@
   return (int)((((const uint32_t*)d.chunk_src)[ch >> 2] >> ((ch & 3) * 8)) & 0xffu);
 }
 
-template <int WC, int WN, int NF, bool AFF, bool DEEP, int R0 = -1, int C0 = -1, bool PART = false>
+template <int WC, int WN, int NF, bool AFF, bool DEEP, int R0 = -1, int C0 = -1, bool PART = false, bool DUAL = false>
 __global__ __launch_bounds__(256, 2) void wgrad3_kernel(const Wg3Args ka) {
   typedef bf16_t T;
   const ksmi_wgrad_desc& d = ka.d;
@@ -72,6 +72,7 @@
   const int xpl = ka.xpl, stage = ka.stage;
 
   const unsigned char* sp[CPT];
+  const unsigned char* sp2[CPT];
   uint32_t cb[CPT];
   bool cvalid[CPT];
   int cc0[CPT], klen[CPT], krem[CPT];
@@ -83,11 +84,13 @@
     const ksmi_src& sr = d.src[wg_chunk_src(d, chs)];
     cc0[c] = wg_chunk_c0(d, chs);
     sp[c] = (const unsigned char*)((const T*)sr.ptr + sr.c_off + cc0[c]);
+    sp2[c] = DUAL ? (const unsigned char*)((const T*)d.seg_ptr + sr.c_off + cc0[c]) : sp[c];
     cb[c] = (uint32_t)sr.C * 2u;
     krem[c] = PART ? sr.c_len - cc0[c] : 32;
     klen[c] = krem[c] >= 32 ? 32 : ((krem[c] + 7) & ~7);
   }
   const unsigned char* const dyp = (const unsigned char*)((const T*)d.dy + d.dy_c_off);
+  const unsigned char* const dyp2 = DUAL ? (const unsigned char*)((const T*)d.seg_dy + d.dy_c_off) : dyp;
   const uint32_t dycb = (uint32_t)d.dyC * 2u;
 
   for (int i = tid * 16; i < ka.lds_bytes; i += 256 * 16) *(u32x4*)(smem + i) = (u32x4){0u, 0u, 0u, 0u};
@@ -100,6 +103,10 @@
       const bool ok = cvalid[c] && (!PART || j < krem[c]);
       aff_tab[tid * 2 + 0] = ok ? sr.scale[cc0[c] + j] : 0.f;
       aff_tab[tid * 2 + 1] = ok ? sr.shift[cc0[c] + j] : 0.f;
+      if constexpr (DUAL) {
+        aff_tab[CPT * 64 + tid * 2 + 0] = ok ? d.seg_scale[cc0[c] + j] : 0.f;
+        aff_tab[CPT * 64 + tid * 2 + 1] = ok ? d.seg_shift[cc0[c] + j] : 0.f;
+      }
     }
   }
   const bool aff_relu = AFF && d.src[0].relu != 0;
@@ -151,6 +158,8 @@
   auto issue_loads = [&](int patch, int stg) {
     int b, oy0, ox0;
     patch_origin(patch, b, oy0, ox0);
+    const bool seg1 = DUAL && b >= d.seg_B;
+    if constexpr (DUAL) b = seg1 ? b - d.seg_B : b;
 #pragma unroll
     for (int it = 0; it < XIT; ++it) {
       const int v = it * 256 + tid;
@@ -169,7 +178,7 @@
         for (int c = 0; c < CPT; ++c) {
           if (!cvalid[c]) continue;
           const bool okc = PART ? (ok && sgr * 8 < klen[c]) : ok;
-          const uint64_t av = (uint64_t)(uintptr_t)sp[c] + (uint64_t)(pix * cb[c] + slb);
+          const uint64_t av = (uint64_t)(uintptr_t)(seg1 ? sp2[c] : sp[c]) + (uint64_t)(pix * cb[c] + slb);
           const uint32_t lo = okc ? (uint32_t)av : zlo, hi = okc ? (uint32_t)(av >> 32) : zhi;
           if (inr) glds16_flat((const unsigned char*)(uintptr_t)(((uint64_t)hi << 32) | lo),
                                lds0 + (unsigned)(stg * stage + c * xpl + (it * 256 + wave * 64) * 16));
@@ -188,7 +197,7 @@
       for (int j = 0; j < NPL; ++j) {
         const int n = n0 + j * 32 + sl * 8;
         const bool okn = pv && n < d.N;
-        const uint64_t av = (uint64_t)(uintptr_t)dyp + (uint64_t)(pix * dycb + (uint32_t)(n * 2));
+        const uint64_t av = (uint64_t)(uintptr_t)(seg1 ? dyp2 : dyp) + (uint64_t)(pix * dycb + (uint32_t)(n * 2));
         const uint32_t lo = okn ? (uint32_t)av : zlo, hi = okn ? (uint32_t)(av >> 32) : zhi;
         glds16_flat((const unsigned char*)(uintptr_t)(((uint64_t)hi << 32) | lo),
                     lds0 + (unsigned)(stg * stage + CPT * xpl + j * 8192 + (it * 256 + wave * 64) * 16));
@@ -199,13 +208,14 @@
     int b, oy0, ox0;
     patch_origin(patch, b, oy0, ox0);
     unsigned char* const sb = smem + stg * stage;
+    const float* const tab = (DUAL && b >= d.seg_B) ? aff_tab + CPT * 64 : aff_tab;
     const int sl = tid & 3;
 #pragma unroll
     for (int c = 0; c < CPT; ++c) {
       if (!cvalid[c]) continue;
       float sc[8], sh[8];
 #pragma unroll
-      for (int j = 0; j < 8; ++j) { sc[j] = aff_tab[(c * 32 + sl * 8 + j) * 2]; sh[j] = aff_tab[(c * 32 + sl * 8 + j) * 2 + 1]; }
+      for (int j = 0; j < 8; ++j) { sc[j] = tab[(c * 32 + sl * 8 + j) * 2]; sh[j] = tab[(c * 32 + sl * 8 + j) * 2 + 1]; }
 #pragma unroll
       for (int it = 0; it < XIT; ++it) {
         const int v = it * 256 + tid;
@@ -429,6 +439,13 @@
   return true;
 }
 
+bool ksmi_wgrad3_dual_ok(const ksmi_wgrad_desc* d, const ksmi_wgrad3_geom_t* g) {
+  if (g->r0 >= 0 || d->nsrc != 1 || d->B < 2) return false;
+  if (d->seg_B != 0 && (d->seg_B < 0 || d->seg_B >= d->B)) return false;
+  if ((d->src[0].c_len % 32) == 0) return true;
+  return g->WC == 2 && g->NTL == 32 && d->src[0].scale == nullptr;
+}
+
 int ksmi_wgrad3_reduce(const ksmi_wgrad_desc* d, const ksmi_wgrad3_geom_t* g, hipStream_t st) {
   const int ntaps = g->r0 >= 0 ? 4 : 9;
   const size_t total4 = (size_t)ntaps * d->nchunks * 32 * ((d->N + 15) & ~15) / 4;
@@ -455,6 +472,26 @@
   if ((size_t)g->patches * 1 >= ((size_t)1 << 31) / 1024) return ksmi_fail(KSMI_E_UNSUPPORTED, "wgrad3: too many patches");
   const dim3 grid(g->nsplit * g->KT * g->NTt);
   const bool aff = d->src[0].scale != nullptr;
+  if (d->seg_B != 0) {
+    if (!ksmi_wgrad3_dual_ok(d, g)) return ksmi_fail(KSMI_E_UNSUPPORTED, "wgrad3: no two-segment instance (ksmi_conv_wgrad_dual_supported)");
+    if (!d->seg_ptr || !d->seg_dy || (aff ? (!d->src[0].shift || !d->seg_scale || !d->seg_shift) : (d->seg_scale || d->seg_shift)))
+      return ksmi_fail(KSMI_E_ARG, "wgrad3: the second segment needs its source, its dy and the same kind of affine as the first");
+#define KSMI_W3D(WC_, WN_, NF_, AFF_, PART_)                                                         \
+  do {                                                                                               \
+    auto kfn = wgrad3_kernel<WC_, WN_, NF_, AFF_, true, -1, -1, PART_, true>; KSMI_NOTE(kfn);        \
+    if (g->lds > 65536) (void)hipFuncSetAttribute((const void*)kfn, hipFuncAttributeMaxDynamicSharedMemorySize, (int)g->lds); \
+    hipLaunchKernelGGL(kfn, grid, dim3(256), g->lds, st, ka);                                        \
+  } while (0)
+#define KSMI_W3DA(WC_, WN_, NF_) do { if (aff) KSMI_W3D(WC_, WN_, NF_, true, false); else KSMI_W3D(WC_, WN_, NF_, false, false); } while (0)
+    if ((d->src[0].c_len % 32) != 0) KSMI_W3D(2, 2, 1, false, true);
+    else if (g->WC == 4 && g->NTL == 64) KSMI_W3DA(4, 1, 4);
+    else if (g->WC == 4) KSMI_W3DA(4, 1, 2);
+    else if (g->NTL == 64) KSMI_W3DA(2, 2, 2);
+    else KSMI_W3DA(2, 2, 1);
+#undef KSMI_W3DA
+#undef KSMI_W3D
+    return ksmi_check_launch("wgrad3");
+  }
   static const bool deep = (ksmi_knob_int("KSMI_WGRAD3_DEEP", 1) != 0);
 #define KSMI_W3_(WC_, WN_, NF_, AFF_, DEEP_)                                                          \
   do {                                                                                               \
diff --git a/kurosiwo_amd/functional.py b/kurosiwo_amd/functional.py
--- a/kurosiwo_amd/functional.py
+++ b/kurosiwo_amd/functional.py
@@ -3,7 +3,7 @@
 import torch
 
 from . import _lib
-from .runtime import DT, SrcSpec, conv_grid_m, conv_npad, conv_stats_rows, make_conv, make_pack, make_wgrad, packed_weight_numel, require_gpu, stream_ptr
+from .runtime import DT, SrcSpec, conv_grid_m, conv_npad, conv_stats_rows, make_conv, make_pack, make_wgrad, packed_weight_numel, require_gpu, set_wgrad_segment, stream_ptr, wgrad_dual_supported
 
 
 def to_nhwc(x_nchw, dtype):
@@ -86,6 +86,39 @@
     d.partial = wsb.data_ptr()
     _lib.check(_lib.load().ksmi_conv_wgrad(C.byref(d), DT[dtype], stream_ptr()), "conv_wgrad")
     return grad
+
+
+def conv3x3_wgrad_dual(x0, dy0, x1, dy1, affine0=None, affine1=None, c_len=None):
+    dtype = dy0.dtype
+    B, H, W, N = dy0.shape
+    assert x0.shape == x1.shape and dy0.shape == dy1.shape and (affine0 is None) == (affine1 is None)
+    Cx = x0.shape[3]
+    K = Cx if c_len is None else c_len
+    src = SrcSpec(x0, Cx, 0, K)
+    if affine0 is not None:
+        src.scale, src.shift, src.relu = affine0
+    grad = torch.zeros((N, K, 3, 3), dtype=torch.float32, device=dy0.device)
+    d, ws = make_wgrad([src], dy0, N, 0, N, grad, 9, K * 9, 1, 0, 2 * B, H, W, H, W, 3, 3, 1, 1, dtype)
+    if not wgrad_dual_supported(d, dtype):
+        raise _lib.KsmiError("conv3x3_wgrad_dual: no two-segment kernel for this shape")
+    set_wgrad_segment(d, B, x1, dy1, *(affine1[:2] if affine1 is not None else ()))
+    wsb = torch.empty(max(ws, 16), dtype=torch.uint8, device=dy0.device)
+    d.partial = wsb.data_ptr()
+    _lib.check(_lib.load().ksmi_conv_wgrad(C.byref(d), DT[dtype], stream_ptr()), "conv_wgrad")
+    return grad
+
+
+def first_nhwc(x, mean=None, std=None, clamp=None, tail=None, dtype=torch.bfloat16):
+    B, ch, H, W = x.shape
+    cin = ch + (tail.shape[1] if tail is not None else 0)
+    cpad = -(-cin // 8) * 8
+    out = torch.empty((B, H, W, cpad), dtype=dtype, device=x.device)
+    t = lambda v: None if v is None else torch.as_tensor(v, dtype=torch.float32, device=x.device)
+    m, s, c = t(mean), t(std), t(clamp)
+    p = lambda v: None if v is None else v.data_ptr()
+    _lib.check(_lib.load().ksmi_first_nhwc_raw(x.data_ptr(), p(tail), ch, out.data_ptr(), B, cin, H, W, cpad, p(m), p(s), p(c), DT[dtype],
+                                               stream_ptr()), "first_nhwc_raw")
+    return out
 
 
 def deconv2x2(x, weight, bias):
diff --git a/kurosiwo_amd/runtime.py b/kurosiwo_amd/runtime.py
--- a/kurosiwo_amd/runtime.py
+++ b/kurosiwo_amd/runtime.py
@@ -273,3 +273,15 @@
     slab = (KH * KW) * len(table) * kc * npad * 4
     d.nsplit = ws // slab
     return d, ws
+
+
+def wgrad_dual_supported(d, dtype):
+    return bool(_lib.load().ksmi_conv_wgrad_dual_supported(C.byref(d), DT[dtype]))
+
+
+def set_wgrad_segment(d, seg_B, tensor, dy, scale=None, shift=None):
+    d.seg_B = seg_B
+    d.seg_ptr, d.seg_dy = tensor.data_ptr(), dy.data_ptr()
+    d.seg_scale = scale.data_ptr() if scale is not None else None
+    d.seg_shift = shift.data_ptr() if shift is not None else None
+    return d
diff --git a/kurosiwo_amd/snunet_plan.py b/kurosiwo_amd/snunet_plan.py
--- a/kurosiwo_amd/snunet_plan.py
+++ b/kurosiwo_amd/snunet_plan.py
@@ -5,7 +5,8 @@
 
 from . import _lib
 from .plan_base import PlanBase, _Saved
-from .runtime import Act, SrcSpec, conv_npad, conv_stats_rows, make_conv, make_pack, make_wgrad, packed_weight_numel
+from .runtime import (Act, SrcSpec, conv_npad, conv_stats_rows, make_conv, make_pack, make_wgrad, packed_weight_numel, set_wgrad_segment,
+                      wgrad_dual_supported)
 from .snunet import BN_EPS, BN_MOMENTUM
 
 
@@ -14,6 +15,8 @@
     two_lanes = True
     bn_fused = os.environ.get("KSMI_BN_FUSED", "1") != "0"
     im2col_late = os.environ.get("KSMI_IM2COL_LATE", "1") != "0"
+    wgrad_dual = os.environ.get("KSMI_WGRAD_DUAL", "1") != "0"
+    first_nhwc = os.environ.get("KSMI_FIRST_NHWC", "1") != "0"
     up_gemm = os.environ.get("KSMI_UP_GEMM", "1") != "0"
     up_wgrad64 = os.environ.get("KSMI_UP_WGRAD64", "1") != "0"
     up_wgrad128 = os.environ.get("KSMI_UP_WGRAD128", "1") != "0"
@@ -40,6 +43,8 @@
         self.logits = torch.empty((B, 3, H, W), dtype=torch.float32, device=self.dev)
         self.dlogits = torch.empty_like(self.logits) if with_backward else None
         self.bwd_builders = []
+        self._siamese = ("conv0_0", "conv1_0", "conv2_0", "conv3_0")
+        self._dual_open = {}
 
         def A(name, lvl, ch):
             return Act(name, B, H >> lvl, W >> lvl, ch, dtype, self.dev)
@@ -164,6 +169,25 @@
         meta["side_ix"] = six
         self.bwd.add("ksmi_conv_wgrad", lambda: (C.byref(d), self.dt), meta)
         self._mark(key)
+
+    def _wgrad_shared(self, name, branch, key, srcs, dy, Cc, gK, gN, gT, B, H, W):
+        dual = self.wgrad_dual and name in self._siamese and self.dtype == torch.bfloat16
+        if dual and branch == "B":
+            d, ws = make_wgrad(srcs, dy, Cc, 0, Cc, self.m._g(key), gK, gN, gT, 0, 2 * B, H, W, H, W, 3, 3, 1, 1, self.dtype)
+            if wgrad_dual_supported(d, self.dtype):
+                self._dual_open[key] = (d, ws)
+                return False
+        if dual and branch == "A" and key in self._dual_open:
+            d, ws = self._dual_open.pop(key)
+            s = srcs[0]
+            set_wgrad_segment(d, B, s.tensor, dy, s.scale, s.shift)
+            d.accumulate = self._acc_param(key)
+            assert d.accumulate == 0 and len(srcs) == 1
+            self._wgrad(d, ws, key)
+            return True
+        d, ws = make_wgrad(srcs, dy, Cc, 0, Cc, self.m._g(key), gK, gN, gT, self._acc_param(key), B, H, W, H, W, 3, 3, 1, 1, self.dtype)
+        self._wgrad(d, ws, key)
+        return True
 
     def _emit_dgrad(self, act, bias_key=None, gate=None):
         cons = getattr(act, "consumers", [])
@@ -325,7 +349,18 @@
             raw = m._raw_ptrs(self.dev)
             self.fwd.add("ksmi_conv_first_forward_raw", lambda: (x_img.data_ptr(), x_tail, chead, P("conv1.weight"), P("conv1.bias"),
                                                                  i_act.t.data_ptr(), stats(), B, cin, H, W, Cc, *raw, dt))
-            if self.with_backward:
+            first_nhwc = False
+            if self.with_backward and self.wgrad_dual and self.first_nhwc and dtype == torch.bfloat16 and cin <= 32 and name in self._siamese:
+                cp8 = -(-cin // 8) * 8
+                img = torch.empty((B, H, W, cp8), dtype=dtype, device=self.dev)
+                probe, _ = make_wgrad([SrcSpec(img, cp8, 0, cin)], i_act.t, Cc, 0, Cc, m._g(f"{name}.conv1.weight"), 9, cin * 9, 1, 0,
+                                      2 * B, H, W, H, W, 3, 3, 1, 1, dtype)
+                first_nhwc = wgrad_dual_supported(probe, dtype)
+                if first_nhwc:
+                    self.keep.append(img)
+                    nhwc_args = lambda: (x_img.data_ptr(), x_tail, chead, img.data_ptr(), B, cin, H, W, cp8, *raw, dt)
+                    src1 = [SrcSpec(img, cp8, 0, cin)]
+            if self.with_backward and not first_nhwc:
                 col = torch.empty((B, H, W, Kpad), dtype=dtype, device=self.dev)
                 self.keep.append(col)
                 im2col_args = lambda: (x_img.data_ptr(), x_tail, chead, col.data_ptr(), B, cin, H, W, Kpad, *raw, dt)
@@ -450,9 +485,7 @@
                 self._mark(f"{name}.bn1.weight", f"{name}.bn1.bias")
                 if self.sync_bn:
                     self.bwd.add_allreduce(lambda: sums1)
-            dw2, ws2 = make_wgrad(src2, dz, Cc, 0, Cc, m._g(f"{name}.conv2.weight"), 9, Cc * 9, 1,
-                                  self._acc_param(f"{name}.conv2.weight"), B, H, W, H, W, 3, 3, 1, 1, dtype)
-            self._wgrad(dw2, ws2, f"{name}.conv2.weight")
+            self._wgrad_shared(name, branch, f"{name}.conv2.weight", src2, dz, Cc, 9, Cc * 9, 1, B, H, W)
             pb1 = torch.empty(rows * Cc, dtype=torch.float32, device=self.dev)
             if fused:
                 rows_b = min(rows, self.lib.ksmi_bn_fused_max_rows())
@@ -466,8 +499,11 @@
                 self.bwd.add("ksmi_bn_bwd_apply_add", lambda: (r.data_ptr(), gout, i_act.t.data_ptr(), sv1.mean, sv1.rstd,
                                                                P("bn1.weight"), s1p, pb1.data_ptr(), rows, gcount, npix, Cc, dt))
                 self._rowsum_at_end(f"{name}.conv1.bias", pb1, rows, 1, 0, Cc, Cc)
-            a_w1 = self._acc_param(f"{name}.conv1.weight")
-            if first:
+            if first and first_nhwc:
+                self.bwd.add("ksmi_first_nhwc_raw", nhwc_args, {"kind": "first_nhwc_raw", "bytes": B * H * W * (cin * 4 + cp8 * self._es()), "flops": 0})
+                self._wgrad_shared(name, branch, f"{name}.conv1.weight", src1, r, Cc, 9, cin * 9, 1, B, H, W)
+            elif first:
+                a_w1 = self._acc_param(f"{name}.conv1.weight")
                 if self.im2col_late:
                     self.bwd.add("ksmi_im2col3x3_raw", im2col_args, {"kind": "im2col3x3_raw", "bytes": B * H * W * (cin * 4 + Kpad * self._es()), "flops": 0})
                 dw1, ws1 = make_wgrad(src1, r, Cc, 0, Cc, m._g(f"{name}.conv1.weight"), 1, cin * 9, 0, a_w1,
@@ -481,9 +517,7 @@
                 for a in sources:
                     a.consumers.append((r, Cc, f"{name}.conv1.weight", nb, Ktot))
                     nb += a.C
-                dw1, ws1 = make_wgrad(srcs, r, Cc, 0, Cc, m._g(f"{name}.conv1.weight"), 9, Ktot * 9, 1, a_w1,
-                                      B, H, W, H, W, 3, 3, 1, 1, dtype)
-                self._wgrad(dw1, ws1, f"{name}.conv1.weight")
+                self._wgrad_shared(name, branch, f"{name}.conv1.weight", srcs, r, Cc, 9, Ktot * 9, 1, B, H, W)
         self.bwd_builders.append((self.fwd.cur_lane, build_bwd))
         if pool is not None:
             return out, pooled
```

After: 2310 tiles/s, median of 6. About the same (+0.5%).
